# dmitrykoval/vinum

Measured on AMD Instinct MI355X. Metric: rows/sec + achieved HBM GB/s, filter->group-by over 10^9-row Arrow batches, higher is better.
Workload: dtype f64/int64; 1 GPU; configs[2]: SELECT k,sum(v),avg(v) WHERE v>63.9921875 GROUP BY k; N=1e+09 rows/GPU, G=1e+08 int64 keys, s=0.5; rows_per_gpu=1000000000, groups=100000000, group_count_hint=none: the operator samples the keys (what the reference boundary allows), parallelism=batch-sharded x1

## Files before the change

vinum_amd/csrc/vnm_agg.hip:

```cpp
#include <memory>
#include <algorithm>
#include <cmath>
#include <cstdlib>
#include <vector>

#include "vnm_agg.hpp"

namespace vnm {

constexpr uint64_t EMPTY = ~0ULL;
constexpr uint64_t LOCKED = ~0ULL - 1;
constexpr int AGG_BLOCK = 1024;
#ifndef VNM_AGG_R
#define VNM_AGG_R 8
#endif
constexpr int AGG_ROWS_PER_THREAD = VNM_AGG_R;
constexpr int AGG_TILE = AGG_BLOCK * AGG_ROWS_PER_THREAD;
constexpr int AGG_LDS_BUDGET = 128 * 1024;
constexpr int AGG_MAX_PROBES = 48;
constexpr int OG_BLOCK = 256;

struct GTable {
    uint64_t* tag;
    uint64_t* keyw;
// ... 197 lines not shown
            continue;
        }
        if (t == EMPTY) {
            uint64_t expected = EMPTY;
            if (__hip_atomic_compare_exchange_strong(&g.tag[h], &expected, LOCKED, __ATOMIC_RELAXED, __ATOMIC_RELAXED,
                                                     __HIP_MEMORY_SCOPE_AGENT)) {
                for (int i = 0; i < g.kwt; i++) st_agent(&g.keyw[(uint64_t)i * g.stride + h], kw[i]);
                asm volatile("s_waitcnt vmcnt(0)" ::: "memory");
                st_agent(&g.tag[h], tagv);
                atomicAdd(newc, 1u);
                return h;
            }
            continue;
        }
        if (t == LOCKED) continue;
        h = (h + 1) & mask;
    }
}

__device__ __forceinline__ void fold_new(const GTable& g, unsigned* s_new) {
    unsigned v = atomicExch(s_new, 0u);
    if (v) atomicAdd(&g.ctl[2], (unsigned long long)v);
}

__device__ __forceinline__ bool op_value(const AccOp& op, const vnm_dcol* cols, int64_t row, uint64_t* out) {
    if (op.kind == A_COUNT_ROWS) { *out = 1; return true; }
    const vnm_dcol& c = cols[op.col];
    if (!col_valid(c, row)) return false;
    switch (op.kind) {
        case A_COUNT_VALID: *out = 1; return true;
        case A_SUM_F64: *out = (uint64_t)__double_as_longlong(col_f64(c, row)); return true;
        case A_SUM_I64: *out = (uint64_t)col_i64(c, row); return true;
        case A_SUM_LO32: *out = (uint64_t)col_i64(c, row) & 0xFFFFFFFFULL; return true;
        case A_SUM_HI32S: *out = (uint64_t)(col_i64(c, row) >> 32); return true;
        case A_SUM_HI32U: *out = (uint64_t)col_i64(c, row) >> 32; return true;
        default:
            if (type_is_float(c.type)) *out = enc_f64(col_f64(c, row));
            else if (type_is_unsigned(c.type)) *out = (uint64_t)col_i64(c, row);
            else *out = enc_i64(col_i64(c, row));
            return true;
    }
}

__device__ __forceinline__ bool table_has_room(const AggArgs& a, unsigned* s_new) {
    fold_new(a.g, s_new);
    unsigned long long fill = __hip_atomic_load(&a.g.ctl[2], __ATOMIC_RELAXED, __HIP_MEMORY_SCOPE_AGENT);
    if ((int64_t)fill + a.margin > a.fill_limit) {
        __hip_atomic_store(&a.g.ctl[1], 1ULL, __ATOMIC_RELAXED, __HIP_MEMORY_SCOPE_AGENT);
        return false;
    }
    return true;
}

#include "vnm_agg_scan.inc"

#include "vnm_agg_tuple.inc"

#include "vnm_agg_onegroup.inc"

#include "vnm_agg_table.inc"

#include "vnm_agg_part.inc"

#include "vnm_agg_pack.inc"

#include "vnm_agg_dense.inc"

#include "vnm_agg_finalize.inc"

}

using namespace vnm;

struct DensePending {
    DFinalArgs df;
    int tb = 0, levels = 0, p1 = 0, fsplits = 1;
    int64_t nfinal = 0;
    int64_t dstride = 0;
    int64_t rows = 0;
    bool x_known = true;
    uint32_t x_inv = 0, x_exp = 0;
    bool exact_ok() const { return x_known && exact_adds_proved(((unsigned long long)x_exp << 32) | x_inv, rows); }
    std::vector<DSet> sets;
    std::vector<void*> blocks;
    DSet* dsets = nullptr;
    DTabSlot* table = nullptr;
    ~DensePending() { for (void* b : blocks) pool_free(b); pool_free(table); pool_free(dsets); }
};
constexpr size_t DP_MAX_SETS = 512;
struct DScanPending {
    DFinalArgs df{};
    DScanTable t{};
    int slots = 0;
    uint64_t* part_sum = nullptr;
    float* part_lo = nullptr;
    uint32_t* part_cnt = nullptr;
    unsigned long long* flags = nullptr;
    ~DScanPending() { pool_free(t.sum); pool_free(t.lo); pool_free(t.cnt); pool_free(part_sum); pool_free(part_lo); pool_free(part_cnt); pool_free(flags); }
};

struct vnm_agg {
    AggPlan plan;
    FuncOut outs[AGG_MAX_FUNCS];
    int n_funcs = 0;
    int func_col[AGG_MAX_FUNCS];
    int col_first_func[AGG_MAX_COLS];
    bool single = false;
    Predicate pred{};
    bool pred_set = false;
    int pred_op = 0, pred_is_float = 0;
    double pred_dval = 0;
    int64_t pred_ival = 0;
    int64_t hint = 0;
    GTable g{};
    bool have_table = false;
    int64_t rows_seen = 0;
    uint64_t* dkey = nullptr;
    uint64_t* dacc = nullptr;
    int64_t dstride = 0;
    int64_t n_groups = -1;
    std::vector<uint64_t> h_key, h_acc;
    bool host_ready = false;
    uint64_t* run_key = nullptr;
    uint64_t* run_acc = nullptr;
    int64_t run_stride = 0, run_n = 0;
    bool have_run = false;
    bool result_is_run = false;
    bool estimated = false;
    int64_t merge_stride = 0;
    unsigned long long* run_dir = nullptr;
    int64_t run_nfin = 0;
    vnm_agg* inner = nullptr;
    bool pack_tried = false;
    bool key_only_failed = false;
    int dense_state = 0;
    DenseMap dmap{};
    int64_t dense_span = 0;
    uint64_t dense_rlo = 0, dense_rhi = 0;
    bool rank_aligned = false;
    struct DensePending* pending = nullptr;
    double heavy_share = 0.0;
    int key_out_type = -1;
    std::vector<std::pair<int64_t, void*>> widened;
    bool widen_in[AGG_MAX_FUNCS] = {};
    bool any_widen_in = false;
    bool pred_lit_rounded = false;
    int pred_user_is_float = 0;
    double pred_user_dval = 0.0;
    int64_t pred_user_ival = 0;
    int fx_state = 0, fx_qe = 0;
    bool pack_null_seen = false;
    bool pring_off = false;
    bool fx_narrow = false;
    int fxn_state = 0, fxn_qe[3] = {0, 0, 0};
    bool null_inputs_seen = false;
    bool count8_off = false;
    int count_cb = 0;
    struct DScanPending* scan_pending = nullptr;
    bool dense_by_bound = false;
    bool range_given = false;
    int expr_col = -1;
    std::vector<vnm_expr_ins> expr_prog;
    int expr_ncols = 0;
    bool expr_fusable = false;
    bool expr_active = false;
    ExprProg expr_dev{};
    PackParams pack{};
    int c_funcs[AGG_MAX_FUNCS], c_in_types[AGG_MAX_FUNCS], c_in_flags[AGG_MAX_FUNCS], c_in_col_ids[AGG_MAX_FUNCS];
    bool c_has_ids = false;
    TDict tdict{};
    int64_t widest_est = 0;
    unsigned long long* tnext = nullptr;
    bool tuple_mode = false;
    std::vector<vnm_agg*> parts;
    std::vector<std::vector<int>> part_funcs;
    bool split_tried = false;
    bool async = false;
    struct QBatch { int64_t nrows; vnm_dcol key, col, pred; std::vector<vnm_dcol> ins; int64_t seq; };
    bool q_multi = false;
    std::vector<QBatch> q;
    int64_t q_rows = 0;
    bool q_pred_is_v = false;
    const std::vector<QBatch>* segs_active = nullptr;
    const uint8_t* kn_valid = nullptr;
    int64_t kn_off = 0;
    bool kn_failed = false;
    std::vector<VSeg> seg_host;
    struct vnm_agg_exact* ex = nullptr;
    bool child = false;
    int64_t seq = 0;
    int64_t cur_seq = -1;
};

namespace {

int table_alloc(vnm_agg* h, GTable* g, uint64_t cap, hipStream_t s) {
    memset(g, 0, sizeof(*g));
    g->cap = cap;
    g->stride = cap + 2;
    g->kwt = h->single || h->plan.n_keys == 0 ? 0 : h->plan.n_keys + 1;
    g->n_words = h->plan.n_words;
    g->tag = (uint64_t*)pool_alloc(g->stride * 8);
    g->acc = (uint64_t*)pool_alloc(g->stride * 8 * (size_t)g->n_words);
    g->ctl = (unsigned long long*)pool_alloc(64);
    if (g->kwt) g->keyw = (uint64_t*)pool_alloc(g->stride * 8 * (size_t)g->kwt);
    if (!g->tag || !g->acc || !g->ctl || (g->kwt && !g->keyw)) return 1;
    VNM_HIP(hipMemsetAsync(g->tag, 0xFF, g->stride * 8, s));
    VNM_HIP(hipMemsetAsync(g->ctl, 0, 64, s));
    for (int w = 0; w < g->n_words; w++) {
        const uint64_t init = merge_init(h->plan.merge[w]);
        if (init == 0 || init == ~0ULL) VNM_HIP(hipMemsetAsync(g->acc + (size_t)w * g->stride, init ? 0xFF : 0, g->stride * 8, s));
        else {
            fill_u64_kernel<<<(int)std::min<uint64_t>((g->stride + 255) / 256, (uint64_t)device_info().num_cus * 8), 256, 0, s>>>(g->acc + (size_t)w * g->stride, init, (int64_t)g->stride);
            VNM_HIP(hipGetLastError());
        }
    }
    return 0;
}

void table_free(GTable* g) {
    pool_free(g->tag);
    pool_free(g->acc);
    pool_free(g->keyw);
    pool_free(g->ctl);
    memset(g, 0, sizeof(*g));
}

uint64_t pow2_at_least(uint64_t x) {
    uint64_t p = 1;
    while (p < x) p <<= 1;
    return p;
}

int lds_slots_for(const AggPlan& p, int budget = AGG_LDS_BUDGET) {
    int per_slot = 8 * (1 + p.n_words);
    int s = 1;
    while ((s * 2 + 2) * per_slot <= budget) s *= 2;
    if (s > 8192) s = 8192;
    return s;
}

int table_grow(vnm_agg* h, uint64_t new_cap, hipStream_t s) {
    GTable old = h->g, ng;
    VNM_TRY(table_alloc(h, &ng, new_cap, s));
    MergeArgs m{};
    m.plan = h->plan;
    m.g = ng;
    m.n = (int64_t)old.stride;
    m.src_is_table = 1;
    m.src_stride = 1;
    m.src_tag = old.tag;
    m.src_cap = (int64_t)old.cap;
    for (int j = 0; j < old.kwt; j++) m.src_key[j] = old.keyw + (size_t)j * old.stride;
    for (int w = 0; w < old.n_words; w++) m.src_acc[w] = old.acc + (size_t)w * old.stride;
    int grid = device_info().num_cus * 8;
    agg_merge_kernel<<<grid, 256, 0, s>>>(m);
    VNM_HIP(hipGetLastError());
    VNM_HIP(hipStreamSynchronize(s));
    table_free(&old);
    h->g = ng;
    return 0;
}

int ensure_table(vnm_agg* h, int64_t nrows, hipStream_t s, bool rows_only = false) {
    if (h->have_table) return 0;
    uint64_t cap;
    if (h->plan.n_keys == 0) cap = 2;
    else {
        uint64_t want = h->hint > 0 ? (uint64_t)h->hint * 2 : (uint64_t)1 << 22;
        if ((h->hint <= 0 || rows_only) && (uint64_t)nrows * 2 < want) want = (uint64_t)(nrows > 512 ? nrows : 512) * 2;
        if (rows_only && want > (1ULL << 20)) want = 1ULL << 20;
        cap = pow2_at_least(want < 1024 ? 1024 : want);
    }
    VNM_TRY(table_alloc(h, &h->g, cap, s));
    h->have_table = true;
    return 0;
}

void invalidate_result(vnm_agg* h) {
    if (!h->result_is_run) {
        pool_free(h->dkey);
        pool_free(h->dacc);
    }
    h->result_is_run = false;
    h->dkey = h->dacc = nullptr;
    h->n_groups = -1;
    h->host_ready = false;
}

int64_t env_i64(const char* name, int64_t dflt) {
    const char* v = getenv(name);
    return v ? (int64_t)atoll(v) : dflt;
}

void drop_run(vnm_agg* h) {
    pool_free(h->run_key);
    pool_free(h->run_acc);
    pool_free(h->run_dir);
    h->run_dir = nullptr;
    h->run_nfin = 0;
    h->run_key = h->run_acc = nullptr;
    h->have_run = false;
    h->run_n = h->run_stride = 0;
}

int estimate_groups(vnm_agg* h, const vnm_dcol& key, int64_t nrows, int64_t* est, hipStream_t s, int64_t* tier0_lb = nullptr) {
// ... 866 lines not shown
```

vinum_amd/csrc/vnm_agg_dense.inc:

```

constexpr int DP_TBITS_MIN = 11, DP_TBITS_MAX = 13;
constexpr int DP_MAX_BITS = DP_TBITS_MAX + 18;

struct DenseMap {
    uint64_t lo_u;
    uint64_t sign;
    uint32_t mul;
    uint32_t mul_inv;
    uint32_t mask;
    int bits;
};

__device__ __forceinline__ uint64_t dense_key_of(const DenseMap& m, uint32_t codep) {
    const uint32_t code = (codep * m.mul_inv) & m.mask;
    return (m.lo_u + code) ^ m.sign;
}

struct DPartArgs {
    DenseMap map;
    const uint64_t* kp;
    const double* vp;
    const double* pp;
    int has_pred, pred_is_v, op;
    double thr;
    int64_t nrows;
    const VSeg* segs;
    int nseg;
    int64_t nsub;
    const double* vp2;
    const double* in_vals2;
    double* out_vals2;
    const uint8_t* kvalid;
    int64_t koff;
    uint64_t* nk_tag;
    uint64_t* nk_rows;
    uint64_t* nk_valid;
    uint64_t* nk_sum;
    int64_t nk_lo_stride;
    int has_expr;
    ExprProg expr;
    const double* in_vals;
    const uint32_t* in_codes;
    const uint32_t* in_counts;
    int64_t in_cap;
    int in_regions, in_split;
    int64_t in_pstride, in_rstride;
    int nt_store;
    int ready_list;
    int producer_major;
    int in_bits;
    double* out_vals;
    void* out_codes;
    uint32_t* out_counts;
    int64_t out_cap;
    int nparts;
    int out_bits;
    int in_pairs;
    unsigned long long* flags;
    ulonglong2* spill;
    int64_t spill_cap;
    const uint8_t* vvalid;
    int64_t voff;
    uint64_t* nspill;
    int64_t nspill_cap;
    double fx_q, fx_inv_q;
    int64_t fx_lim;
};
constexpr uint32_t DP_NULL32 = 0x80000000u;
__device__ __forceinline__ bool fx_encode(double v, double inv_q, int64_t* m, int64_t lim = 2147483647LL) {
    const double MAGIC = 6755399441055744.0;
    const double t = v * inv_q;
    const double u = t + MAGIC;
    const int64_t mm = (int64_t)(__double_as_longlong(u) - __double_as_longlong(MAGIC));
    *m = mm;
    return (u - MAGIC == t) && mm >= -lim && mm <= lim && __double_as_longlong(v) != (long long)0x8000000000000000ULL;
}
__device__ __forceinline__ double fx_bits(int64_t m) { return __longlong_as_double((long long)m); }
__device__ __forceinline__ int64_t fx_of(double carried) { return (int64_t)__double_as_longlong(carried); }
__device__ __forceinline__ void fx_expand(int64_t total, double q, double* hi, double* lo) {
    const double h = (double)total;
    const double l = (double)(total - (int64_t)h);
    *hi = h * q; *lo = l * q;
}

__device__ __forceinline__ void dense_spill(const DPartArgs& a, uint64_t key, double v, bool isnull = false) {
    if (isnull) {
        const unsigned long long pos = atomicAdd(&a.flags[3], 1ULL);
        if ((int64_t)pos < a.nspill_cap) a.nspill[pos] = key;
        else __hip_atomic_store(&a.flags[0], 1ULL, __ATOMIC_RELAXED, __HIP_MEMORY_SCOPE_AGENT);
        return;
    }
    const unsigned long long pos = atomicAdd(&a.flags[2], 1ULL);
    if ((int64_t)pos < a.spill_cap) a.spill[pos] = make_ulonglong2(key, (unsigned long long)__double_as_longlong(v));
    else __hip_atomic_store(&a.flags[0], 1ULL, __ATOMIC_RELAXED, __HIP_MEMORY_SCOPE_AGENT);
}
__device__ __forceinline__ void dense_spill_wave(const DPartArgs& a, bool want, uint64_t key, double v) {
    const unsigned long long m = __ballot(want);
    if (!m) return;
    const int lane = threadIdx.x & 63;
    const int leader = __ffsll((long long)m) - 1;
    unsigned long long base = 0;
    if (lane == leader) base = atomicAdd(&a.flags[2], (unsigned long long)__popcll(m));
    base = __shfl(base, leader);
    if (want) {
        const unsigned long long pos = base + (unsigned long long)__popcll(m & ((1ULL << lane) - 1ULL));
        if ((int64_t)pos < a.spill_cap) a.spill[pos] = make_ulonglong2(key, (unsigned long long)__double_as_longlong(v));
        else __hip_atomic_store(&a.flags[0], 1ULL, __ATOMIC_RELAXED, __HIP_MEMORY_SCOPE_AGENT);
    }
}
template <typename CT>
__device__ __forceinline__ CT dense_rem(uint32_t c, uint32_t remmask) {
    return (CT)((c & remmask) | ((c >> 31) << (sizeof(CT) * 8 - 1)));
}
template <typename CT>
__device__ __forceinline__ uint32_t dense_rem_code(CT r) { return (uint32_t)r & ((1u << (sizeof(CT) * 8 - 1)) - 1u); }
template <typename CT>
__device__ __forceinline__ bool dense_rem_null(CT r) { return ((uint32_t)r >> (sizeof(CT) * 8 - 1)) != 0; }

template <bool FROM_ROWS, typename CT, bool HAS_VAL = true, bool VN = false>
__global__ __launch_bounds__(PT_BLOCK) void dpart_scatter_kernel(DPartArgs a) {
    __shared__ double stage_v[HAS_VAL ? PT_TILE : 1];
    __shared__ uint32_t stage_c[PT_TILE];
    __shared__ uint32_t cnt[PT_MAXP], off[PT_MAXP], cursor[PT_MAXP];
    __shared__ uint32_t s_total;
    __shared__ uint32_t wtot[PT_MAXP / 64];
    const int tid = threadIdx.x;
    const int lane = tid & 63;
    const int np = a.nparts;
    const int npad = np < 64 ? 64 : np;
    const uint32_t remmask = (1u << a.out_bits) - 1u;
    for (int i = tid; i < PT_MAXP; i += PT_BLOCK) { cnt[i] = 0; cursor[i] = 0; }
    __syncthreads();

    int64_t out_base, out_stride;
    int64_t ntiles = 0;
    uint32_t prefix = 0;
    if (FROM_ROWS) {
        if (a.producer_major) { out_base = (int64_t)blockIdx.x * np; out_stride = 1; }
        else { out_base = blockIdx.x; out_stride = gridDim.x; }
        ntiles = (a.nrows + PT_TILE - 1) / PT_TILE;
    } else {
        const int pin = blockIdx.x / a.in_split, g = blockIdx.x % a.in_split;
        out_base = (int64_t)pin * np * a.in_split + g; out_stride = a.in_split;
        prefix = (uint32_t)pin << a.in_bits;
    }
    double* const ov = a.out_vals;
    CT* const oc = (CT*)a.out_codes;

    auto process_tile = [&](auto&& get_item, auto&& prefetch_next) {
        uint32_t myc[PT_ITEMS], myr[PT_ITEMS];
        double myv[PT_ITEMS];
#pragma unroll
        for (int k = 0; k < PT_ITEMS; k++) {
            myr[k] = 0xFFFFFFFFu;
            uint32_t c; double v;
            if (get_item(k, &c, &v)) {
                myc[k] = c;
                if (HAS_VAL) myv[k] = v;
                myr[k] = atomicAdd(&cnt[(c & ~DP_NULL32) >> a.out_bits], 1u);
            }
        }
        prefetch_next();
        __syncthreads();
        if (tid < npad) {
            uint32_t c = cnt[tid], inc = c;
#pragma unroll
            for (int d = 1; d < 64; d <<= 1) { uint32_t o = __shfl_up(inc, d); if (lane >= d) inc += o; }
            off[tid] = inc - c;
            if (lane == 63) wtot[tid >> 6] = inc;
        }
        __syncthreads();
        if (tid < npad) {
            uint32_t add = 0;
            for (int w = 0; w < (tid >> 6); w++) add += wtot[w];
            off[tid] += add;
            if (tid == npad - 1) s_total = off[tid] + cnt[tid];
        }
        __syncthreads();
#pragma unroll
        for (int k = 0; k < PT_ITEMS; k++) {
            if (myr[k] != 0xFFFFFFFFu) {
                const uint32_t pos = off[(myc[k] & ~DP_NULL32) >> a.out_bits] + myr[k];
                if (HAS_VAL) stage_v[pos] = myv[k];
                stage_c[pos] = myc[k];
            }
        }
        __syncthreads();
        const uint32_t total = s_total;
#pragma unroll
        for (int q = 0; q < PT_ITEMS; q++) {
            const uint32_t i = (uint32_t)q * PT_BLOCK + tid;
            bool lost = false;
            uint32_t c = 0;
            if (i < total) {
                c = stage_c[i];
                const uint32_t p = (c & ~DP_NULL32) >> a.out_bits;
                const uint32_t j = cursor[p] + (i - off[p]);
                if (j < (uint32_t)a.out_cap) {
                    const int64_t at = (out_base + (int64_t)p * out_stride) * a.out_cap + j;
                    if (a.nt_store) {
                        if (HAS_VAL) __builtin_nontemporal_store(stage_v[i], &ov[at]);
                        __builtin_nontemporal_store(dense_rem<CT>(c, remmask), &oc[at]);
                    } else {
                        if (HAS_VAL) ov[at] = stage_v[i];
                        oc[at] = dense_rem<CT>(c, remmask);
                    }
                } else lost = true;
            }
            if (lost && (c >> 31)) { dense_spill(a, dense_key_of(a.map, prefix | (c & ~DP_NULL32)), 0.0, true); lost = false; }
            dense_spill_wave(a, lost, dense_key_of(a.map, prefix | (c & ~DP_NULL32)), HAS_VAL && lost ? stage_v[i] : 0.0);
        }
        __syncthreads();
        if (tid < np) { cursor[tid] += cnt[tid]; cnt[tid] = 0; }
        __syncthreads();
    };

    if (FROM_ROWS) {
        ulonglong2 kk[PT_PAIRS];
        double2 vv[PT_PAIRS], pv[PT_PAIRS];
        uint8_t vb[VN ? PT_PAIRS : 1];
        auto load_rows = [&](int64_t tile) {
            const int64_t base = tile * PT_TILE;
            if (tile < ntiles && base + PT_TILE <= a.nrows) {
#pragma unroll
                for (int u = 0; u < PT_PAIRS; u++) {
                    const int64_t r = base + (int64_t)u * 2 * PT_BLOCK + 2 * tid;
                    kk[u] = *(const ulonglong2*)(a.kp + r);
                    if (HAS_VAL) vv[u] = a.has_expr ? expr_eval2(a.expr, r) : *(const double2*)(a.vp + r);
                    if (a.has_pred && !a.pred_is_v) pv[u] = *(const double2*)(a.pp + r);
                    if (VN) vb[VN ? u : 0] = (uint8_t)(a.vvalid[(a.voff + r) >> 3] >> ((a.voff + r) & 7));
                }
            }
        };
        load_rows(blockIdx.x);
        for (int64_t tile = blockIdx.x; tile < ntiles; tile += gridDim.x) {
            const int64_t base = tile * PT_TILE;
            const bool full = base + PT_TILE <= a.nrows;
            process_tile([&](int k, uint32_t* c, double* v) -> bool {
                const int u = k >> 1, el = k & 1;
                const int64_t r = base + (int64_t)u * 2 * PT_BLOCK + 2 * tid + el;
                if (r >= a.nrows) return false;
                uint64_t key; double val, p;
                bool isnull = false;
                if (full) {
                    key = el ? kk[u].y : kk[u].x;
                    val = HAS_VAL ? (el ? vv[u].y : vv[u].x) : 0.0;
                    p = a.pred_is_v ? val : (a.has_pred ? (el ? pv[u].y : pv[u].x) : 0.0);
                    if (VN) isnull = !((vb[VN ? u : 0] >> el) & 1);
                } else {
                    key = a.kp[r]; val = HAS_VAL ? (a.has_expr ? expr_eval1(a.expr, r) : a.vp[r]) : 0.0; p = a.has_pred ? (a.pred_is_v ? val : a.pp[r]) : 0.0;
                    if (VN) isnull = !((a.vvalid[(a.voff + r) >> 3] >> ((a.voff + r) & 7)) & 1);
                }
                if (VN && isnull && a.pred_is_v) return false;
                if (a.has_pred && !cmp_apply<double>(a.op, p, a.thr)) return false;
                const uint64_t d = (key ^ a.map.sign) - a.map.lo_u;
                if (d > (uint64_t)a.map.mask) { dense_spill(a, key, val, isnull); return false; }
                *c = (((uint32_t)d * a.map.mul) & a.map.mask) | (isnull ? DP_NULL32 : 0u);
                *v = isnull ? 0.0 : val;
                return true;
            }, [&]() { load_rows(tile + gridDim.x); });
        }
    } else {
        __shared__ uint32_t rstart[PT_MAX_REGIONS + 1];
        const int pin = blockIdx.x / a.in_split;
        const int per_max = (a.in_regions + a.in_split - 1) / a.in_split;
        const int g = blockIdx.x % a.in_split;
        const int first = g * per_max;
        const int per = first + per_max <= a.in_regions ? per_max : (a.in_regions > first ? a.in_regions - first : 0);
        const int64_t region0 = (int64_t)pin * a.in_pstride + (int64_t)first * a.in_rstride;
        if (tid == 0) {
            uint32_t run = 0;
            for (int rj = 0; rj < per; rj++) { rstart[rj] = run; run += (a.in_counts[region0 + rj * a.in_rstride] + 1) / 2; }
            rstart[per] = run;
        }
        __syncthreads();
        const uint32_t total_in = rstart[per];
        double2 ev[PT_PAIRS];
        uint2 ec[PT_PAIRS];
        uint32_t ok[PT_PAIRS];
        int reg[PT_PAIRS];
#pragma unroll
        for (int k = 0; k < PT_PAIRS; k++) reg[k] = 0;
        auto load_entries = [&](uint32_t t0) {
#pragma unroll
            for (int k = 0; k < PT_PAIRS; k++) {
                const uint32_t v = t0 + (uint32_t)k * PT_BLOCK + tid;
                ok[k] = 0;
                if (v < total_in) {
                    int lo = reg[k];
                    while (rstart[lo + 1] <= v) lo++;
                    reg[k] = lo;
                    const uint32_t e0 = 2u * (v - rstart[lo]);
                    const int64_t rg = region0 + lo * a.in_rstride;
                    const int64_t at = rg * a.in_cap + e0;
                    if (HAS_VAL) ev[k] = *(const double2*)(a.in_vals + at);
                    ec[k] = *(const uint2*)(a.in_codes + at);
                    ok[k] = e0 + 1 < a.in_counts[rg] ? 3u : 1u;
                }
            }
        };
        load_entries(0);
        for (uint32_t t0 = 0; t0 < total_in; t0 += PT_TILE / 2) {
            process_tile([&](int k, uint32_t* c, double* v) -> bool {
                const int u = k >> 1, el = k & 1;
                if (!((ok[u] >> el) & 1u)) return false;
                *c = el ? ec[u].y : ec[u].x;
                *v = HAS_VAL ? (el ? ev[u].y : ev[u].x) : 0.0;
                return true;
            }, [&]() { load_entries(t0 + PT_TILE / 2); });
        }
    }
    if (tid < np) a.out_counts[out_base + (int64_t)tid * out_stride] = cursor[tid] < (uint32_t)a.out_cap ? cursor[tid] : (uint32_t)a.out_cap;
}

__device__ __forceinline__ void exact_track(double v, uint32_t& xinv, uint32_t& xexp) {
    const uint64_t b = (uint64_t)__double_as_longlong(v) & 0x7FFFFFFFFFFFFFFFULL;
    if (b == 0) return;
    const uint32_t hi = (uint32_t)(b >> 32), lo = (uint32_t)b;
    const uint32_t e = hi >> 20;
    const uint32_t mh = (hi & 0xFFFFFu) | (e ? 0x100000u : 0u);
    const uint32_t tz = lo ? (uint32_t)__builtin_ctz(lo) : 32u + (uint32_t)__builtin_ctz(mh);
    const uint32_t low = (e ? e : 1u) + tz;
    xinv = max(xinv, 0xFFFFu - low);
    xexp = max(xexp, e);
}
static inline bool exact_adds_proved(unsigned long long word, int64_t rows) {
    const uint32_t xinv = (uint32_t)word, xexp = (uint32_t)(word >> 32);
    if (xinv == 0 && xexp == 0) return true;
    if (xexp >= 2047) return false;
    int lg = 0;
    while (((int64_t)1 << lg) < rows) lg++;
    return (int64_t)lg + (int64_t)xexp <= (int64_t)(0xFFFFu - xinv);
}

constexpr int DR_FB = 16;
typedef double dr_v2 __attribute__((ext_vector_type(2)));
typedef uint32_t dr_u2 __attribute__((ext_vector_type(2)));
template <bool FROM_ROWS, typename CT, bool HAS_VAL, int DR_BLOCK, int DR_PAIRS, bool PV = false, bool VN = false, int MAXR = 0, bool SEG = false, bool KN = false,
          bool V2 = false, bool FX = false, bool W32 = false>
__global__ __launch_bounds__(DR_BLOCK) void dring_scatter_kernel(DPartArgs a, int ring_cap) {
    extern __shared__ uint64_t dr_lds[];
    static_assert(!FX || (HAS_VAL && !V2), "fixed-point entries: one value (VN: only where the filter drops the NULL rows, vn_fold)");
    static_assert(!W32 || FX, "32-bit entry words are fixed-point words");
    constexpr int FB = W32 ? 32 : DR_FB, EPL = FB / 8;
    constexpr int NE = 2 * DR_PAIRS;
    const int np = a.nparts;
    double* const rv = (double*)dr_lds;
    double* const rv2 = rv + (V2 ? (size_t)np * ring_cap : 0);
    CT* const rc = (CT*)(dr_lds + (HAS_VAL ? (size_t)np * ring_cap * (V2 ? 2 : 1) : 0));
    __shared__ uint32_t fill[PT_MAXP], head[PT_MAXP], cursor[PT_MAXP];
    __shared__ uint32_t s_retry[2];
    __shared__ uint32_t s_nready[2];
    __shared__ uint16_t ready[2][PT_MAXP];
    __shared__ uint32_t s_spill[3];
    const int tid = threadIdx.x;
    const uint32_t remmask = (1u << a.out_bits) - 1u;
    for (int i = tid; i < PT_MAXP; i += DR_BLOCK) { fill[i] = 0; head[i] = 0; cursor[i] = 0; }
    if (tid < 2) { s_retry[tid] = 0; s_nready[tid] = 0; }
    int ph = 0;
    const bool use_list = a.ready_list != 0;
    if (tid == 0) s_spill[0] = 0;
    __syncthreads();

    int64_t out_base, out_stride;
    uint32_t prefix = 0;
    if (FROM_ROWS) {
        if (a.producer_major) { out_base = (int64_t)blockIdx.x * np; out_stride = 1; }
        else { out_base = blockIdx.x; out_stride = gridDim.x; }
    } else {
        const int pin = blockIdx.x / a.in_split, g = blockIdx.x % a.in_split;
        out_base = (int64_t)pin * np * a.in_split + g; out_stride = a.in_split;
        prefix = (uint32_t)pin << a.in_bits;
    }
    double* const ov = a.out_vals;
    double* const ov2 = a.out_vals2;
    CT* const oc = (CT*)a.out_codes;
    const uint32_t ocap = (uint32_t)a.out_cap;

    auto insert = [&](uint32_t c, double v, double w2) -> bool {
        const uint32_t p = (c & ~DP_NULL32) >> a.out_bits;
        const uint32_t r = atomicAdd(&fill[p], 1u);
        if (r == (uint32_t)FB - 1u && use_list) ready[ph][atomicAdd(&s_nready[ph], 1u)] = (uint16_t)p;
        if (r >= (uint32_t)ring_cap) return false;
        uint32_t slot = head[p] + r;
        if (slot >= (uint32_t)ring_cap) slot -= ring_cap;
        if (W32) {
            ((uint32_t*)rv)[(size_t)p * ring_cap + slot] = ((uint32_t)(int32_t)fx_of(v) << a.out_bits) | (c & remmask);
            return true;
        }
        if (FX) {
            ((uint64_t*)rv)[(size_t)p * ring_cap + slot] = ((uint64_t)fx_of(v) << a.out_bits) | (uint64_t)(c & remmask);
            return true;
        }
        if (HAS_VAL) rv[(size_t)p * ring_cap + slot] = v;
        if (V2) rv2[(size_t)p * ring_cap + slot] = w2;
        rc[(size_t)p * ring_cap + slot] = dense_rem<CT>(c, remmask);
        return true;
    };
    auto fx_rem = [&](size_t li) -> uint32_t { return W32 ? ((const uint32_t*)rv)[li] & remmask : (uint32_t)(((const uint64_t*)rv)[li] & (uint64_t)remmask); };
    auto fx_val = [&](size_t li) -> double {
        return W32 ? (double)((int32_t)((const uint32_t*)rv)[li] >> a.out_bits) * a.fx_q : (double)((int64_t)((const uint64_t*)rv)[li] >> a.out_bits) * a.fx_q;
    };
    auto flush = [&](bool drain) {
        const int j = tid & 7;
        const bool listed = use_list && !drain;
        const int nwalk = listed ? (int)s_nready[ph] : np;
        for (int q = tid >> 3; q < nwalk; q += DR_BLOCK / 8) {
            const int p = listed ? (int)ready[ph][q] : q;
            uint32_t f = fill[p];
            if (f > (uint32_t)ring_cap) f = ring_cap;
            const uint32_t nb = drain ? (f + FB - 1) / FB : f / FB;
            if (nb == 0) continue;
            const uint32_t h = head[p], cur = cursor[p];
            const int64_t rbase = (out_base + (int64_t)p * out_stride) * a.out_cap;
            uint32_t done = 0, wrote = 0;
            for (uint32_t b = 0; b < nb; b++) {
                uint32_t src = h + b * FB;
                if (src >= (uint32_t)ring_cap) src -= ring_cap;
                const uint32_t n_here = f - b * FB < (uint32_t)FB ? f - b * FB : FB;
                const size_t li = (size_t)p * ring_cap + src + EPL * j;
                if (cur + wrote + FB <= ocap) {
                    const int64_t at = rbase + cur + wrote + EPL * j;
                    if ((uint32_t)(EPL * j) < n_here) {
                        if (W32) {
                            const dr_v2 x = *(const dr_v2*)((const uint32_t*)rv + li);
                            if (a.nt_store) __builtin_nontemporal_store(x, (dr_v2*)((uint32_t*)ov + at)); else *(dr_v2*)((uint32_t*)ov + at) = x;
                        } else if (HAS_VAL) {
                            const dr_v2 x = *(const dr_v2*)(rv + li);
                            if (a.nt_store) __builtin_nontemporal_store(x, (dr_v2*)(ov + at)); else *(dr_v2*)(ov + at) = x;
                        }
                        if (V2) {
                            const dr_v2 x2 = *(const dr_v2*)(rv2 + li);
                            if (a.nt_store) __builtin_nontemporal_store(x2, (dr_v2*)(ov2 + at)); else *(dr_v2*)(ov2 + at) = x2;
                        }
                        if (FX) {
                        } else if (sizeof(CT) == 4) {
                            const dr_u2 y = *(const dr_u2*)(rc + li);
                            if (a.nt_store) __builtin_nontemporal_store(y, (dr_u2*)(oc + at)); else *(dr_u2*)(oc + at) = y;
                        } else {
                            const uint32_t y = *(const uint32_t*)(rc + li);
                            if (a.nt_store) __builtin_nontemporal_store(y, (uint32_t*)(oc + at)); else *(uint32_t*)(oc + at) = y;
                        }
                    }
                    wrote += n_here;
                } else if (V2) {
                    if (j == 0) __hip_atomic_store(&a.flags[0], 1ULL, __ATOMIC_RELAXED, __HIP_MEMORY_SCOPE_AGENT);
                } else if (!drain && a.nspill == nullptr) {
                    const unsigned long long m = __ballot(j == 0);
                    const int lane = tid & 63;
                    const int leader = __ffsll((long long)m) - 1;
                    unsigned long long base = 0;
                    if (lane == leader) base = atomicAdd(&a.flags[2], (unsigned long long)__popcll(m) * FB);
                    base = __shfl(base, leader);
                    const unsigned long long pos = base + (unsigned long long)__popcll(m & ((1ULL << (lane - j)) - 1ULL)) * FB + EPL * j;
                    if ((int64_t)(pos + EPL) <= a.spill_cap) {
                        for (int e = 0; e < EPL; e++)
                            a.spill[pos + e] = make_ulonglong2(dense_key_of(a.map, prefix | (p << a.out_bits) | (FX ? fx_rem(li + e) : dense_rem_code<CT>(rc[FX ? 0 : li + e]))),
                                                               (unsigned long long)__double_as_longlong(FX ? fx_val(li + e) : (HAS_VAL ? rv[li + e] : 0.0)));
                    } else __hip_atomic_store(&a.flags[0], 1ULL, __ATOMIC_RELAXED, __HIP_MEMORY_SCOPE_AGENT);
                } else {
                    for (int e = 0; e < EPL; e++)
                        if ((uint32_t)(EPL * j + e) < n_here) {
                            if (FX) dense_spill(a, dense_key_of(a.map, prefix | (p << a.out_bits) | fx_rem(li + e)), fx_val(li + e));
                            else dense_spill(a, dense_key_of(a.map, prefix | (p << a.out_bits) | dense_rem_code<CT>(rc[FX ? 0 : li + e])), HAS_VAL ? rv[li + e] : 0.0,
                                             dense_rem_null<CT>(rc[FX ? 0 : li + e]));
                        }
                }
                done += n_here;
            }
            if (j == 0) {
                uint32_t nh = h + nb * FB;
                while (nh >= (uint32_t)ring_cap) nh -= ring_cap;
                head[p] = drain ? 0 : nh;
                fill[p] = f - done;
                cursor[p] = cur + wrote;
            }
        }
    };
    int maxr = MAXR;
    auto rounds = [&](const uint32_t (&c)[NE], const double (&v)[NE], const double (&w2)[V2 ? NE : 1], uint32_t okmask) {
        uint32_t pend = 0;
        int nr = 0;
#pragma unroll
        for (int e = 0; e < NE; e++) if (((okmask >> e) & 1u) && !insert(c[e], v[e], w2[V2 ? e : 0])) pend |= 1u << e;
        for (;;) {
            if (pend) s_retry[ph] = 1;
            __syncthreads();
            flush(false);
            if (tid == 0) { s_retry[ph ^ 1] = 0; s_nready[ph ^ 1] = 0; }
            __syncthreads();
            const bool again = s_retry[ph] != 0;
            ph ^= 1;
            if (!again) break;
            if (MAXR > 0 && ++nr >= maxr) {
                uint32_t mine = 0;
#pragma unroll
                for (int e = 0; e < NE; e++) {
                    if (((pend >> e) & 1u) && (c[e] >> 31)) {
                        dense_spill(a, dense_key_of(a.map, prefix | (c[e] & ~DP_NULL32)), 0.0, true);
                        pend &= ~(1u << e);
                    }
                }
                mine = (uint32_t)__popc(pend);
                uint32_t at = mine ? atomicAdd(&s_spill[0], mine) : 0u;
                __syncthreads();
                if (tid == 0) {
                    const unsigned long long base = atomicAdd(&a.flags[2], (unsigned long long)s_spill[0]);
                    s_spill[1] = (uint32_t)base; s_spill[2] = (uint32_t)(base >> 32);
                }
                __syncthreads();
                const unsigned long long base = ((unsigned long long)s_spill[2] << 32) | s_spill[1];
#pragma unroll
                for (int e = 0; e < NE; e++) {
                    if ((pend >> e) & 1u) {
                        const unsigned long long pos = base + at++;
                        if ((int64_t)pos < a.spill_cap)
                            a.spill[pos] = make_ulonglong2(dense_key_of(a.map, prefix | c[e]),
                                                           (unsigned long long)__double_as_longlong(FX ? (double)fx_of(v[e]) * a.fx_q : (HAS_VAL ? v[e] : 0.0)));
                        else __hip_atomic_store(&a.flags[0], 1ULL, __ATOMIC_RELAXED, __HIP_MEMORY_SCOPE_AGENT);
                    }
                }
                __syncthreads();
                if (tid == 0) s_spill[0] = 0;
                maxr = MAXR - 1;
                break;
            }
#pragma unroll
            for (int e = 0; e < NE; e++) if (((pend >> e) & 1u) && insert(c[e], v[e], w2[V2 ? e : 0])) pend &= ~(1u << e);
        }
    };

    double nk_hi = -0.0, nk_lo = 0.0;
    uint32_t nk_cnt = 0;
    constexpr bool XT = FROM_ROWS && HAS_VAL && !V2 && !FX;
    uint32_t xinv = 0, xexp = 0;
    bool fx_bad = false;
    if (FROM_ROWS && !SEG) {
        const int64_t sub = (int64_t)NE * DR_BLOCK;
        const int64_t nsub = (a.nrows + sub - 1) / sub;
        const int64_t nfull = a.nrows / sub;
        ulonglong2 kk[DR_PAIRS];
        double2 vv[DR_PAIRS], pv[PV ? DR_PAIRS : 1], vv2[V2 ? DR_PAIRS : 1];
        uint32_t vbits = 0;
        uint32_t kbits = 0;
        auto load_sub = [&](int64_t st) {
            if (st < nfull) {
                if (VN) vbits = 0;
                if (KN) kbits = 0;
#pragma unroll
                for (int u = 0; u < DR_PAIRS; u++) {
                    const int64_t r = st * sub + (int64_t)u * 2 * DR_BLOCK + 2 * tid;
                    kk[u] = *(const ulonglong2*)(a.kp + r);
                    if (HAS_VAL) vv[u] = *(const double2*)(a.vp + r);
                    if (V2) vv2[V2 ? u : 0] = *(const double2*)(a.vp2 + r);
                    if (PV) pv[u] = *(const double2*)(a.pp + r);
                    if (VN) vbits |= (((uint32_t)a.vvalid[(a.voff + r) >> 3] >> ((a.voff + r) & 7)) & 3u) << (2 * u);
                    if (KN) kbits |= (((uint32_t)a.kvalid[(a.koff + r) >> 3] >> ((a.koff + r) & 7)) & 3u) << (2 * u);
                }
            }
        };
        load_sub(blockIdx.x);
        for (int64_t st = blockIdx.x; st < nsub; st += gridDim.x) {
            uint32_t c[NE]; double v[NE]; double w2[V2 ? NE : 1]; uint32_t okmask = 0;
#pragma unroll
            for (int e = 0; e < NE; e++) {
                const int u = e >> 1, el = e & 1;
                const int64_t r = st * sub + (int64_t)u * 2 * DR_BLOCK + 2 * tid + el;
                c[e] = 0; v[e] = 0.0;
                if (r >= a.nrows) continue;
                uint64_t key; double val, p, val2 = 0.0;
                bool isnull = false, keynull = false;
                if (st < nfull) {
                    if (KN) keynull = !((kbits >> e) & 1u);
                    key = el ? kk[u].y : kk[u].x;
                    val = HAS_VAL ? (el ? vv[u].y : vv[u].x) : 0.0;
                    if (V2) val2 = el ? vv2[V2 ? u : 0].y : vv2[V2 ? u : 0].x;
                    p = PV ? (el ? pv[PV ? u : 0].y : pv[PV ? u : 0].x) : val;
                    if (VN) isnull = !((vbits >> e) & 1u);
                } else {
                    key = a.kp[r]; val = HAS_VAL ? a.vp[r] : 0.0; p = a.has_pred ? (a.pred_is_v ? val : a.pp[r]) : 0.0;
                    if (V2) val2 = a.vp2[r];
                    if (VN) isnull = !((a.vvalid[(a.voff + r) >> 3] >> ((a.voff + r) & 7)) & 1);
                    if (KN) keynull = !((a.kvalid[(a.koff + r) >> 3] >> ((a.koff + r) & 7)) & 1);
                }
                if (VN && isnull && a.pred_is_v) continue;
                if (a.has_pred && !cmp_apply<double>(a.op, p, a.thr)) continue;
                if (KN && keynull) {
                    nk_cnt++;
                    const double t = nk_hi + val;
                    nk_lo += two_sum_err(nk_hi, val, t);
                    nk_hi = t;
                    continue;
                }
                const uint64_t d = (key ^ a.map.sign) - a.map.lo_u;
                if (d > (uint64_t)a.map.mask) {
                    if (V2) __hip_atomic_store(&a.flags[0], 1ULL, __ATOMIC_RELAXED, __HIP_MEMORY_SCOPE_AGENT);
                    else dense_spill(a, key, val, isnull);
                    continue;
                }
                c[e] = (((uint32_t)d * a.map.mul) & a.map.mask) | (VN && isnull ? DP_NULL32 : 0u);
                v[e] = VN && isnull ? 0.0 : val;
                if (FX) { int64_t m; if (!fx_encode(val, a.fx_inv_q, &m, a.fx_lim)) { fx_bad = true; continue; } v[e] = fx_bits(m); }
                if (V2) w2[V2 ? e : 0] = val2;
                if (XT) exact_track(v[e], xinv, xexp);
                okmask |= 1u << e;
            }
            load_sub(st + gridDim.x);
            rounds(c, v, w2, okmask);
        }
    } else if (FROM_ROWS) {
        const int64_t sub = (int64_t)NE * DR_BLOCK;
        struct Cur { const uint64_t* kp; const double* vp; const double* pp; const uint8_t* vvalid; int64_t voff; int64_t nrows; int64_t lst; };
        const int nseg = a.nseg;
        const VSegConst segs = seg_table(a.segs);
        const int64_t nsub = a.nsub;
        int sg = 0;
        auto locate = [&](int64_t st, Cur& c) {
            while (sg + 1 < nseg && st >= segs[sg + 1].first_tile) sg++;
            c.kp = segs[sg].kp; c.vp = (const double*)segs[sg].vp; c.pp = segs[sg].pp;
            c.vvalid = VN ? segs[sg].vvalid : nullptr; c.voff = VN ? segs[sg].voff : 0;
            c.nrows = segs[sg].nrows;
            c.lst = st - segs[sg].first_tile;
        };
        ulonglong2 kk[DR_PAIRS];
        double2 vv[DR_PAIRS], pv[PV ? DR_PAIRS : 1];
        uint32_t vbits = 0;
        auto load_sub = [&](const Cur& c) {
            if (c.lst < c.nrows / sub) {
                if (VN) vbits = 0;
#pragma unroll
                for (int u = 0; u < DR_PAIRS; u++) {
                    const int64_t r = c.lst * sub + (int64_t)u * 2 * DR_BLOCK + 2 * tid;
                    kk[u] = *(const ulonglong2*)(c.kp + r);
                    if (HAS_VAL) vv[u] = *(const double2*)(c.vp + r);
                    if (PV) pv[u] = *(const double2*)(c.pp + r);
                    if (VN) vbits |= (((uint32_t)c.vvalid[(c.voff + r) >> 3] >> ((c.voff + r) & 7)) & 3u) << (2 * u);
                }
            }
        };
        Cur cur{}, nxt{};
        if ((int64_t)blockIdx.x < nsub) { locate(blockIdx.x, cur); load_sub(cur); }
        for (int64_t st = blockIdx.x; st < nsub; st += gridDim.x) {
            uint32_t c[NE]; double v[NE]; uint32_t okmask = 0;
            const bool full = cur.lst < cur.nrows / sub;
#pragma unroll
            for (int e = 0; e < NE; e++) {
                const int u = e >> 1, el = e & 1;
                const int64_t r = cur.lst * sub + (int64_t)u * 2 * DR_BLOCK + 2 * tid + el;
                c[e] = 0; v[e] = 0.0;
                if (r >= cur.nrows) continue;
                uint64_t key; double val, p;
                bool isnull = false;
                if (full) {
                    key = el ? kk[u].y : kk[u].x;
                    val = HAS_VAL ? (el ? vv[u].y : vv[u].x) : 0.0;
                    p = PV ? (el ? pv[PV ? u : 0].y : pv[PV ? u : 0].x) : val;
                    if (VN) isnull = !((vbits >> e) & 1u);
                } else {
                    key = cur.kp[r]; val = HAS_VAL ? cur.vp[r] : 0.0; p = a.has_pred ? (a.pred_is_v ? val : cur.pp[r]) : 0.0;
                    if (VN) isnull = !((cur.vvalid[(cur.voff + r) >> 3] >> ((cur.voff + r) & 7)) & 1);
                }
                if (VN && isnull && a.pred_is_v) continue;
                if (a.has_pred && !cmp_apply<double>(a.op, p, a.thr)) continue;
                const uint64_t d = (key ^ a.map.sign) - a.map.lo_u;
                if (d > (uint64_t)a.map.mask) { dense_spill(a, key, val, isnull); continue; }
                c[e] = (((uint32_t)d * a.map.mul) & a.map.mask) | (VN && isnull ? DP_NULL32 : 0u);
                v[e] = VN && isnull ? 0.0 : val;
                if (FX) { int64_t m; if (!fx_encode(val, a.fx_inv_q, &m, a.fx_lim)) { fx_bad = true; continue; } v[e] = fx_bits(m); }
                if (XT) exact_track(v[e], xinv, xexp);
                okmask |= 1u << e;
            }
            if (st + gridDim.x < nsub) { locate(st + gridDim.x, nxt); load_sub(nxt); }
            const double w2[V2 ? NE : 1] = {};
            rounds(c, v, w2, okmask);
            cur = nxt;
        }
    } else {
        __shared__ uint32_t rstart[PT_MAX_REGIONS + 1];
        const int pin = blockIdx.x / a.in_split;
        const int per_max = (a.in_regions + a.in_split - 1) / a.in_split;
        const int g = blockIdx.x % a.in_split;
        const int first = g * per_max;
        const int per = first + per_max <= a.in_regions ? per_max : (a.in_regions > first ? a.in_regions - first : 0);
        const int64_t region0 = (int64_t)pin * a.in_pstride + (int64_t)first * a.in_rstride;
        if (tid == 0) {
            uint32_t run = 0;
            for (int rj = 0; rj < per; rj++) { rstart[rj] = run; run += (a.in_counts[region0 + rj * a.in_rstride] + 1) / 2; }
            rstart[per] = run;
        }
        __syncthreads();
        const uint32_t total_in = rstart[per];
        double2 ev[DR_PAIRS], ev2[V2 ? DR_PAIRS : 1];
        uint2 ec[DR_PAIRS];
        uint32_t okm = 0;
        int reg = 0;
        auto load_pairs = [&](uint32_t t0) {
            okm = 0;
#pragma unroll
            for (int u = 0; u < DR_PAIRS; u++) {
                const uint32_t v = t0 + (uint32_t)u * DR_BLOCK + tid;
                if (v < total_in) {
                    int lo = reg;
                    while (rstart[lo + 1] <= v) lo++;
                    reg = lo;
                    const uint32_t e0 = 2u * (v - rstart[lo]);
                    const int64_t rg = region0 + lo * a.in_rstride;
                    const int64_t at = rg * a.in_cap + e0;
                    if (HAS_VAL) ev[u] = *(const double2*)(a.in_vals + at);
                    if (V2) ev2[V2 ? u : 0] = *(const double2*)(a.in_vals2 + at);
                    if (!FX) ec[u] = *(const uint2*)(a.in_codes + at);
                    okm |= (e0 + 1 < a.in_counts[rg] ? 3u : 1u) << (2 * u);
                }
            }
        };
        load_pairs(0);
        for (uint32_t t0 = 0; t0 < total_in; t0 += DR_PAIRS * DR_BLOCK) {
            uint32_t c[NE]; double v[NE]; double w2[V2 ? NE : 1];
#pragma unroll
            for (int u = 0; u < DR_PAIRS; u++) {
                if (FX) {
                    const uint64_t w0 = (uint64_t)__double_as_longlong(ev[u].x), w1 = (uint64_t)__double_as_longlong(ev[u].y);
                    const uint64_t inmask = ((uint64_t)1 << a.in_bits) - 1;
                    c[2 * u] = (uint32_t)(w0 & inmask); c[2 * u + 1] = (uint32_t)(w1 & inmask);
                    v[2 * u] = fx_bits((int64_t)w0 >> a.in_bits); v[2 * u + 1] = fx_bits((int64_t)w1 >> a.in_bits);
                    continue;
                }
                c[2 * u] = ec[u].x; c[2 * u + 1] = ec[u].y;
                v[2 * u] = HAS_VAL ? ev[u].x : 0.0; v[2 * u + 1] = HAS_VAL ? ev[u].y : 0.0;
                if (V2) { w2[V2 ? 2 * u : 0] = ev2[V2 ? u : 0].x; w2[V2 ? 2 * u + 1 : 0] = ev2[V2 ? u : 0].y; }
            }
            const uint32_t okmask = okm;
            load_pairs(t0 + DR_PAIRS * DR_BLOCK);
            rounds(c, v, w2, okmask);
        }
    }
    flush(true);
    __syncthreads();
    if (tid < np) a.out_counts[out_base + (int64_t)tid * out_stride] = cursor[tid];
    if (FX && FROM_ROWS) { if (__syncthreads_or(fx_bad ? 1 : 0) && tid == 0) __hip_atomic_store(&a.flags[7], 1ULL, __ATOMIC_RELAXED, __HIP_MEMORY_SCOPE_AGENT); }
    if (XT) {
        if (tid < 2) s_spill[tid] = 0;
        __syncthreads();
        if (xinv) atomicMax(&s_spill[0], xinv);
        if (xexp) atomicMax(&s_spill[1], xexp);
        __syncthreads();
        if (tid < 2 && s_spill[tid]) atomicMax((uint32_t*)&a.flags[6] + tid, s_spill[tid]);
    }
    if (KN) {
        __shared__ uint64_t s_nk[3];
        __syncthreads();
        if (tid < 3) s_nk[tid] = tid == 0 ? F64_NEG_ZERO : 0;
        __syncthreads();
        if (nk_cnt) {
            l_add_f64c(&s_nk[0], 1, nk_hi);
            __hip_atomic_fetch_add((double*)&s_nk[1], nk_lo, __ATOMIC_RELAXED, __HIP_MEMORY_SCOPE_WORKGROUP);
            __hip_atomic_fetch_add(&s_nk[2], (uint64_t)nk_cnt, __ATOMIC_RELAXED, __HIP_MEMORY_SCOPE_WORKGROUP);
        }
        __syncthreads();
        if (tid == 0 && s_nk[2]) {
            if (ld_agent(a.nk_tag) == EMPTY) st_agent(a.nk_tag, 0);
            if (a.nk_rows) __hip_atomic_fetch_add(a.nk_rows, s_nk[2], __ATOMIC_RELAXED, __HIP_MEMORY_SCOPE_AGENT);
            if (a.nk_valid) __hip_atomic_fetch_add(a.nk_valid, s_nk[2], __ATOMIC_RELAXED, __HIP_MEMORY_SCOPE_AGENT);
            if (a.nk_sum) {
                if (a.nk_lo_stride) {
                    g_add_f64c(a.nk_sum, a.nk_lo_stride, __longlong_as_double((long long)s_nk[0]));
                    __hip_atomic_fetch_add((double*)(a.nk_sum + a.nk_lo_stride), __longlong_as_double((long long)s_nk[1]), __ATOMIC_RELAXED, __HIP_MEMORY_SCOPE_AGENT);
                } else __hip_atomic_fetch_add((double*)a.nk_sum, __longlong_as_double((long long)s_nk[0]) + __longlong_as_double((long long)s_nk[1]), __ATOMIC_RELAXED, __HIP_MEMORY_SCOPE_AGENT);
            }
        }
    }
}

__global__ void dnull_fold_kernel(const unsigned long long* scr, uint64_t* tag, uint64_t* rows, uint64_t* valid, uint64_t* sum, int64_t lo_stride) {
    if (threadIdx.x != 0 || blockIdx.x != 0) return;
    if (!(scr[1] | scr[2])) return;
    if (ld_agent(tag) == EMPTY) st_agent(tag, 0);
    if (rows) __hip_atomic_fetch_add(rows, scr[1], __ATOMIC_RELAXED, __HIP_MEMORY_SCOPE_AGENT);
    if (valid) __hip_atomic_fetch_add(valid, scr[2], __ATOMIC_RELAXED, __HIP_MEMORY_SCOPE_AGENT);
    if (sum) {
        if (lo_stride) {
            g_add_f64c(sum, lo_stride, __longlong_as_double((long long)scr[3]));
            __hip_atomic_fetch_add((double*)(sum + lo_stride), __longlong_as_double((long long)scr[4]), __ATOMIC_RELAXED, __HIP_MEMORY_SCOPE_AGENT);
        } else __hip_atomic_fetch_add((double*)sum, __longlong_as_double((long long)scr[3]), __ATOMIC_RELAXED, __HIP_MEMORY_SCOPE_AGENT);
    }
}

struct DSet {
    const double* vals; const void* codes; const uint32_t* counts;
    int64_t cap, pstride, rstride;
    int regions, pad;
};
__device__ __forceinline__ const double* dfin_words(const double* base, int64_t entries, bool w32) {
    return w32 ? (const double*)((const uint32_t*)base + entries) : base + entries;
}
constexpr int DF_MAX_OUT = 8;
enum { DF_RUN = 0, DF_COLS = 1, DF_TABLE = 2 };
enum { DF_KEY = 0, DF_SUM = 1, DF_AVG = 2, DF_COUNT = 3 };
struct DTabSlot { double sum; float lo; uint32_t cnt; };
struct DFinalArgs {
    int64_t pstride, rstride;
    DenseMap map;
    const double* vals;
    const void* codes;
    const uint32_t* counts;
    int64_t cap;
    int regions;
    int64_t nfinal;
    int w_rows, w_valid, w_sum, w_lo;
    uint64_t* dkey;
    uint64_t* dacc;
    int64_t dstride;
    unsigned long long* flags;
    int splits;
    uint64_t* part_sum;
    float* part_lo;
    uint32_t* part_cnt;
    int n_out;
    int out_kind[DF_MAX_OUT];
    int key_width;
    void* out_ptr[DF_MAX_OUT];
    DTabSlot* table;
    const DSet* sets;
    int nsets;
    int sub_bits, sub;
    int has_side;
    GTable side;
    const uint32_t* side_bloom;
    uint32_t side_bloom_mask;
    uint8_t* side_found;
    int64_t* null_pos;
    const double* vals2;
    int w_valid2, w_sum2, w_lo2;
    double fx_q;
    int fx_w32;
    int pack_n;
    int key_field[DF_MAX_OUT];
    int pack_shift[AGG_MAX_KEYS], pack_bits[AGG_MAX_KEYS];
    uint64_t pack_lo[AGG_MAX_KEYS];
};
__device__ __forceinline__ uint64_t df_key_cell(const DFinalArgs& a, int c, uint64_t key) {
    if (!a.pack_n) return key;
    const int f = a.key_field[c];
    return ((key >> a.pack_shift[f]) & ((1ULL << a.pack_bits[f]) - 1ULL)) + a.pack_lo[f];
}
__device__ __forceinline__ void df_store_cell(const DFinalArgs& a, int c, int64_t pos, uint64_t cell) {
    if (a.out_kind[c] == DF_KEY && a.key_width && a.key_width != 8) {
        if (a.key_width == 4) ((uint32_t*)a.out_ptr[c])[pos] = (uint32_t)cell;
        else if (a.key_width == 2) ((uint16_t*)a.out_ptr[c])[pos] = (uint16_t)cell;
        else ((uint8_t*)a.out_ptr[c])[pos] = (uint8_t)cell;
        return;
    }
    ((uint64_t*)a.out_ptr[c])[pos] = cell;
}
constexpr int DSIDE_BLOOM_BITS = 1 << 16;
__device__ __forceinline__ uint32_t dside_bloom_bit(uint64_t k, uint32_t mask) { return hash_u64(k ^ 0xD6E8FEB86659FD93ULL) & mask; }
__device__ __forceinline__ uint32_t dside_bloom_pattern(uint64_t k, uint32_t b) {
    const uint32_t h2 = hash_u64(k * 0x9E3779B97F4A7C15ULL + 0x632BE59BD9B4E019ULL);
    return (1u << (b & 31)) | (1u << ((h2 >> 7) & 31));
}
__device__ __forceinline__ void dside_merge(const DFinalArgs& a, const uint32_t* lb, uint64_t key, double& hi, double& lo, uint64_t& cnt) {
    const GTable& g = a.side;
    uint64_t slot = ~0ULL;
    if (key == EMPTY) { if (g.tag[g.cap] != EMPTY) slot = g.cap; }
    else {
        const uint32_t bb = dside_bloom_bit(key, a.side_bloom_mask);
        const uint32_t word = (lb && a.side_bloom_mask == DSIDE_BLOOM_BITS - 1) ? lb[bb >> 5] : a.side_bloom[bb >> 5];
        const uint32_t pat = dside_bloom_pattern(key, bb);
        if ((word & pat) != pat) return;
        const uint64_t mask = g.cap - 1;
        uint64_t h = hash_u64(key) & mask;
        for (uint64_t probes = 0; probes <= mask; probes++) {
            const uint64_t t = g.tag[h];
            if (t == key) { slot = h; break; }
            if (t == EMPTY) break;
            h = (h + 1) & mask;
        }
    }
    if (slot == ~0ULL) return;
    const int wc = a.w_rows >= 0 ? a.w_rows : a.w_valid;
    if (wc >= 0) cnt += g.acc[(uint64_t)wc * g.stride + slot];
    if (a.w_sum >= 0) {
        const double sh = __longlong_as_double((long long)g.acc[(uint64_t)a.w_sum * g.stride + slot]);
        const double t = hi + sh;
        lo += two_sum_err(hi, sh, t);
        if (a.w_lo >= 0) lo += __longlong_as_double((long long)g.acc[(uint64_t)a.w_lo * g.stride + slot]);
        hi = t;
    }
    a.side_found[slot] = 1;
}
__global__ __launch_bounds__(256) void dside_bloom_kernel(GTable g, uint32_t* bloom, uint32_t bmask) {
    const int64_t stride = (int64_t)gridDim.x * 256;
    for (int64_t slot = (int64_t)blockIdx.x * 256 + threadIdx.x; slot < (int64_t)g.cap; slot += stride) {
// ... 1083 lines not shown
            for (uint32_t i0 = 0; i0 < n; i0 += 64 * 4 * 2) {
                uint4 q[2];
#pragma unroll
                for (int u = 0; u < 2; u++) {
                    const uint32_t i = i0 + ((uint32_t)u * 64 + lane) * 4;
                    if (i < n) q[u] = *(const uint4*)(sc + i);
                }
#pragma unroll
                for (int u = 0; u < 2; u++) {
                    const uint32_t i = i0 + ((uint32_t)u * 64 + lane) * 4;
                    const uint32_t c4[4] = {q[u].x, q[u].y, q[u].z, q[u].w};
#pragma unroll
                    for (int k = 0; k < 4; k++) {
                        if (i + k >= n) continue;
                        const uint32_t code = c4[k];
                        if ((code >> tb8) != sub) continue;
                        const uint32_t b = code & ((1u << tb8) - 1u), sh = (b & (uint32_t)(PER - 1)) * (uint32_t)CB;
                        const uint32_t old = atomicAdd(&dc_tab[b >> PSH], 1u << sh);
                        over |= ((old >> sh) & CMASK) == CMASK;
                    }
                }
            }
        }
        if (over) s_over = 1;
        __syncthreads();
        if (s_over) {
            if (tid == 0) { __hip_atomic_store(&a.flags[5], 1ULL, __ATOMIC_RELAXED, __HIP_MEMORY_SCOPE_AGENT); __hip_atomic_store(&a.flags[0], 1ULL, __ATOMIC_RELAXED, __HIP_MEMORY_SCOPE_AGENT); }
            return;
        }
        uint32_t mine = 0;
        for (int i = tid; i < (1 << (tb8 - PSH)); i += 1024) {
            const uint32_t x = dc_tab[i];
            if (CB == 8) mine += ((x & 0xffu) != 0) + ((x & 0xff00u) != 0) + ((x & 0xff0000u) != 0) + ((x >> 24) != 0);
            else mine += ((x & 0xffffu) != 0) + ((x >> 16) != 0);
        }
        pa_block_add(&s_n, mine);
        __syncthreads();
        const uint32_t ngroups = s_n;
        __syncthreads();
        if (tid == 0) { s_base = atomicAdd(&a.flags[1], (unsigned long long)ngroups); s_n = 0; }
        __syncthreads();
        if ((int64_t)(s_base + ngroups) > a.dstride) {
            if (tid == 0) __hip_atomic_store(&a.flags[0], 1ULL, __ATOMIC_RELAXED, __HIP_MEMORY_SCOPE_AGENT);
            return;
        }
        const uint32_t prefix = ((uint32_t)p << (tb8 + sub_bits)) | (sub << tb8);
        for (int i0 = 0; i0 < (1 << tb8); i0 += 1024) {
            const int i = i0 + tid;
            const uint32_t cnt = (dc_tab[i >> PSH] >> ((i & (PER - 1)) * CB)) & CMASK;
            const bool occ = cnt != 0;
            const uint64_t b = __ballot(occ);
            uint32_t wbase = 0;
            if (lane == 0 && b) wbase = atomicAdd(&s_n, (uint32_t)__popcll(b));
            wbase = __shfl(wbase, 0);
            if (occ) {
                const uint64_t lt = lane == 0 ? 0ULL : (~0ULL >> (64 - lane));
                dgen_write_group(a, (int64_t)s_base + wbase + __popcll(b & lt), prefix | (uint32_t)i, cnt, nullptr);
            }
        }
        __syncthreads();
    }
}

struct DScanTable {
    double* sum;
    double* lo;
    unsigned long long* cnt;
};
__global__ __launch_bounds__(512) void dscan_accumulate_kernel(const uint64_t* part_sum, const float* part_lo, const uint32_t* part_cnt,
                                                                int splits, int slots, DScanTable t) {
    __shared__ double s_hi[8][64], s_lo[8][64];
    __shared__ unsigned long long s_cnt[8][64];
    const int li = threadIdx.x & 63, g = threadIdx.x >> 6;
    const int i = blockIdx.x * 64 + li;
    double hi = -0.0, lo = 0.0;
    unsigned long long cnt = 0;
    constexpr int U = 4;
    for (int sp0 = g; sp0 < splits; sp0 += 8 * U) {
        uint32_t c[U]; uint64_t xs[U]; float xl[U];
#pragma unroll
        for (int u = 0; u < U; u++) {
            const int sp = sp0 + 8 * u;
            c[u] = 0; xs[u] = 0; xl[u] = 0.0f;
            if (sp < splits && i < slots) {
                const size_t at = (size_t)sp * slots + i;
                c[u] = part_cnt[at]; xs[u] = part_sum[at]; xl[u] = part_lo[at];
            }
        }
#pragma unroll
        for (int u = 0; u < U; u++) {
            if (c[u] == 0) continue;
            cnt += c[u];
            const double x = __longlong_as_double((long long)xs[u]);
            const double s = hi + x;
            lo += two_sum_err(hi, x, s) + (double)xl[u];
            hi = s;
        }
    }
    s_hi[g][li] = hi; s_lo[g][li] = lo; s_cnt[g][li] = cnt;
    __syncthreads();
    if (g != 0 || i >= slots) return;
    for (int gg = 1; gg < 8; gg++) {
        const unsigned long long c = s_cnt[gg][li];
        if (c == 0) continue;
        cnt += c;
        const double x = s_hi[gg][li];
        const double s = hi + x;
        lo += two_sum_err(hi, x, s) + s_lo[gg][li];
        hi = s;
    }
    if (cnt == 0) return;
    const double old = t.sum[i], s = old + hi;
    t.lo[i] += two_sum_err(old, hi, s) + lo;
    t.sum[i] = s;
    t.cnt[i] += cnt;
}
__global__ __launch_bounds__(512) void dscan_emit_kernel(DFinalArgs a, int slots, DScanTable t) {
    __shared__ uint32_t s_n;
    __shared__ unsigned long long s_base;
    const int tid = threadIdx.x, lane = tid & 63;
    const int i = blockIdx.x * 512 + tid;
    if (tid == 0) s_n = 0;
    __syncthreads();
    const unsigned long long cnt = i < slots ? t.cnt[i] : 0ULL;
    const bool occ = cnt != 0;
    pa_block_add(&s_n, occ ? 1u : 0u);
    __syncthreads();
    const uint32_t ngroups = s_n;
    __syncthreads();
    if (tid == 0) { s_base = atomicAdd(&a.flags[1], (unsigned long long)ngroups); s_n = 0; }
    __syncthreads();
    if ((int64_t)(s_base + ngroups) > a.dstride) {
        if (tid == 0) __hip_atomic_store(&a.flags[0], 1ULL, __ATOMIC_RELAXED, __HIP_MEMORY_SCOPE_AGENT);
        return;
    }
    const uint64_t b = __ballot(occ);
    uint32_t wbase = 0;
    if (lane == 0 && b) wbase = atomicAdd(&s_n, (uint32_t)__popcll(b));
    wbase = __shfl(wbase, 0);
    if (occ) {
        const uint64_t lt = lane == 0 ? 0ULL : (~0ULL >> (64 - lane));
        const int64_t pos = (int64_t)s_base + wbase + __popcll(b & lt);
        const double hi = t.sum[i], lo = t.lo[i];
        a.dkey[pos] = dense_key_of(a.map, (uint32_t)i);
        a.dkey[a.dstride + pos] = 0;
        if (a.w_rows >= 0) a.dacc[(int64_t)a.w_rows * a.dstride + pos] = cnt;
        if (a.w_valid >= 0) a.dacc[(int64_t)a.w_valid * a.dstride + pos] = cnt;
        if (a.w_sum >= 0) a.dacc[(int64_t)a.w_sum * a.dstride + pos] = (uint64_t)__double_as_longlong(hi);
        if (a.w_lo >= 0) a.dacc[(int64_t)a.w_lo * a.dstride + pos] = (uint64_t)__double_as_longlong(lo);
        else if (a.w_sum >= 0) a.dacc[(int64_t)a.w_sum * a.dstride + pos] = (uint64_t)__double_as_longlong(fsum2(hi, lo));
    }
}

__global__ __launch_bounds__(256) void fx_sample_kernel(const double* vals, int64_t nrows, int64_t m, unsigned long long* out) {
    __shared__ uint32_t sx[2];
    if (threadIdx.x < 2) sx[threadIdx.x] = 0;
    __syncthreads();
    const int64_t stride = (int64_t)gridDim.x * blockDim.x;
    uint32_t xinv = 0, xexp = 0;
    for (int64_t i = (int64_t)blockIdx.x * blockDim.x + threadIdx.x; i < m; i += stride) exact_track(vals[(int64_t)(((__int128)i * nrows) / m)], xinv, xexp);
    if (xinv) atomicMax(&sx[0], xinv);
    if (xexp) atomicMax(&sx[1], xexp);
    __syncthreads();
    if (threadIdx.x < 2 && sx[threadIdx.x]) atomicMax((uint32_t*)out + threadIdx.x, sx[threadIdx.x]);
}

__global__ __launch_bounds__(256) void dense_sample_range_kernel(const uint64_t* keys, int64_t nrows, int64_t m, uint64_t sign,
                                                                 unsigned long long* out, const uint8_t* kvalid, int64_t koff) {
    __shared__ unsigned long long smn[4], smx[4];
    const int64_t stride = (int64_t)gridDim.x * blockDim.x;
    uint64_t mn = ~0ULL, mx = 0;
    for (int64_t i = (int64_t)blockIdx.x * blockDim.x + threadIdx.x; i < m; i += stride) {
        const int64_t row = (int64_t)(((__int128)i * nrows) / m);
        if (!key_row_valid(kvalid, koff, row)) continue;
        const uint64_t ku = keys[row] ^ sign;
        mn = ku < mn ? ku : mn;
        mx = ku > mx ? ku : mx;
    }
#pragma unroll
    for (int o = 32; o > 0; o >>= 1) {
        const uint64_t omn = __shfl_xor(mn, o), omx = __shfl_xor(mx, o);
        mn = omn < mn ? omn : mn;
        mx = omx > mx ? omx : mx;
    }
    if ((threadIdx.x & 63) == 0) { smn[threadIdx.x >> 6] = mn; smx[threadIdx.x >> 6] = mx; }
    __syncthreads();
    if (threadIdx.x == 0) {
        for (int w = 1; w < 4; w++) { mn = smn[w] < mn ? smn[w] : mn; mx = smx[w] > mx ? smx[w] : mx; }
        atomicMin(&out[0], (unsigned long long)mn);
        atomicMax(&out[1], (unsigned long long)mx);
    }
}
```

vinum_amd/csrc/vnm_agg_fxn.inc:

```
constexpr int FXN_MAXV = 3;
constexpr int FXN_BLOCK = 1024;
constexpr int FXN_FB = 16;
typedef uint32_t fxn_u4 __attribute__((ext_vector_type(4)));

struct VSegN { const uint64_t* kp; const double* vp[FXN_MAXV]; const double* pp; int64_t nrows; int64_t first_tile; };
typedef const VSegN __attribute__((address_space(4)))* VSegNConst;

struct FxnArgs {
    DenseMap map;
    const uint64_t* kp;
    const double* vp[FXN_MAXV];
    const double* pp;
    int has_pred, pred_col, op;
    double thr;
    int64_t nrows;
    const VSegN* segs;
    int nseg;
    int64_t nsub;
    double inv_q[FXN_MAXV];
    const fxn_u4* in_ent;
    const uint32_t* in_counts;
    int64_t in_cap;
    int in_regions, in_split;
    int in_bits;
// ... 242 lines not shown
    const int tid = threadIdx.x, lane = tid & 63;
    const int R = a.regions;
    const int64_t nwork = a.nfinal;
    int buf = 0;
    if ((int64_t)blockIdx.x < nwork) for (int r = tid; r < R && r < MAXR; r += BLOCK) s_cnt[0][r] = a.counts[(int64_t)blockIdx.x * R + r];
    __syncthreads();
    auto first_region = [&](const uint32_t* cnt) { int r = 0; while (r < R && cnt[r] == 0) r++; return r; };
    fxn_u4 pa = fxn_u4{0u, 0u, 0u, 0u}, pb = pa;
    uint32_t na = 0, ia = 0, nb = 0, ib = 0;
    auto load_chunk = [&](int64_t f, int rj, uint32_t ci, uint32_t n, fxn_u4* p) {
        const uint32_t i = ci + tid;
        if (i < n) *p = a.ent[(f * R + rj) * a.cap + i];
    };
    int rj = 0; uint32_t ci = 0;
    bool have = false;
    if ((int64_t)blockIdx.x < nwork) {
        rj = first_region(s_cnt[0]);
        have = rj < R;
        if (have) { na = s_cnt[0][rj]; ia = 0; load_chunk(blockIdx.x, rj, 0, na, &pa); ci = BLOCK; }
    }
    for (int64_t w = blockIdx.x; w < nwork; w += gridDim.x) {
        const int64_t f = w, wn = w + gridDim.x;
        for (int i = tid; i < SLOTS; i += BLOCK) {
#pragma unroll
            for (int v = 0; v < NV; v++) lsum[v][i] = 0ULL;
            lcnt[i] = 0;
        }
        if (tid == 0) s_n = 0;
        uint32_t cnext[CQ];
        if (wn < nwork) {
#pragma unroll
            for (int q = 0; q < CQ; q++) { const int r = q * BLOCK + tid; cnext[q] = r < R ? a.counts[wn * R + r] : 0u; }
        }
        __syncthreads();
        const uint32_t* cnt = s_cnt[buf];
        while (have) {
            int rn = rj; uint32_t cin = ci;
            while (rn < R && cin >= cnt[rn]) { rn++; cin = 0; }
            const bool more = rn < R;
            if (more) { nb = cnt[rn]; ib = cin; load_chunk(f, rn, cin, nb, &pb); }
            if (ia + tid < na) {
                const uint32_t slot = pa.w & (SLOTS - 1);
                atomicAdd(&lsum[0][slot], (unsigned long long)(long long)(int32_t)pa.x);
                if (NV > 1) atomicAdd(&lsum[NV > 1 ? 1 : 0][slot], (unsigned long long)(long long)(int32_t)pa.y);
                if (NV > 2) atomicAdd(&lsum[NV > 2 ? 2 : 0][slot], (unsigned long long)(long long)(int32_t)pa.z);
                atomicAdd(&lcnt[slot], 1u);
            }
            have = more;
            if (more) { pa = pb; na = nb; ia = ib; rj = rn; ci = cin + BLOCK; }
        }
        if (wn < nwork) {
#pragma unroll
            for (int q = 0; q < CQ; q++) { const int r = q * BLOCK + tid; if (r < R) s_cnt[buf ^ 1][r] = cnext[q]; }
        }
        __syncthreads();
        if (wn < nwork) {
            const uint32_t* cn2 = s_cnt[buf ^ 1];
            rj = first_region(cn2);
            have = rj < R;
            if (have) { na = cn2[rj]; ia = 0; load_chunk(wn, rj, 0, na, &pa); ci = BLOCK; }
        }
        buf ^= 1;
        uint32_t mine = 0;
#pragma unroll
        for (int q = 0; q < SLOTS / BLOCK; q++) mine += lcnt[q * BLOCK + tid] != 0 ? 1u : 0u;
        pa_block_add(&s_n, mine);
        __syncthreads();
        const uint32_t ngroups = s_n;
        __syncthreads();
        if (tid == 0) { s_base = atomicAdd(&a.flags[1], (unsigned long long)ngroups); s_n = 0; }
        __syncthreads();
        if ((int64_t)(s_base + ngroups) > a.dstride) {
            if (tid == 0) __hip_atomic_store(&a.flags[0], 1ULL, __ATOMIC_RELAXED, __HIP_MEMORY_SCOPE_AGENT);
            return;
        }
        for (int i0 = 0; i0 < SLOTS; i0 += BLOCK) {
            const int i = i0 + tid;
            const uint32_t gc = lcnt[i];
            const bool occ = gc != 0;
            const uint64_t b = __ballot(occ);
            uint32_t wbase = 0;
            if (lane == 0 && b) wbase = atomicAdd(&s_n, (uint32_t)__popcll(b));
            wbase = __shfl(wbase, 0);
            if (occ) {
                const uint64_t lt = lane == 0 ? 0ULL : (~0ULL >> (64 - lane));
                const int64_t pos = (int64_t)s_base + wbase + __popcll(b & lt);
                a.dkey[pos] = dense_key_of(a.map, ((uint32_t)f << TB) | (uint32_t)i);
                a.dkey[a.dstride + pos] = 0;
                for (int k = 0; k < a.n_cnt; k++) a.dacc[(int64_t)a.w_cnt[k] * a.dstride + pos] = gc;
#pragma unroll
                for (int v = 0; v < NV; v++) {
                    if (a.w_sum[v] < 0) continue;
                    double hi, lo;
                    fx_expand((long long)lsum[v][i], a.q[v], &hi, &lo);
                    a.dacc[(int64_t)a.w_sum[v] * a.dstride + pos] = (uint64_t)__double_as_longlong(hi);
                    a.dacc[(int64_t)(a.w_sum[v] + 1) * a.dstride + pos] = (uint64_t)__double_as_longlong(lo);
                }
            }
        }
        __syncthreads();
    }
}

int dense_fxn_aggregate(vnm_agg* h, int64_t nrows, const vnm_dcol* keys, const vnm_dcol* inputs, const vnm_dcol* pred, hipStream_t s) {
    if (env_i64("VNM_DENSE_FXN", 1) == 0 || h->fxn_state < 0) return 2;
    const AggPlan& pl = h->plan;
    const int NV = pl.n_cols;
    if (!h->single || pl.n_keys != 1 || NV < 2 || NV > FXN_MAXV || h->rank_aligned || h->kn_valid || h->expr_col >= 0 || h->dense_state != 1) return 2;
    auto plain8 = [](const vnm_dcol& c) { return !c.validity && (c.offset & 1) == 0 && ((uintptr_t)c.values & 15) == 0; };
    if ((keys[0].type != VNM_I64 && keys[0].type != VNM_U64) || !plain8(keys[0])) return 2;
    FxnFinalArgs fa{};
    for (int v = 0; v < FXN_MAXV; v++) fa.w_sum[v] = -1;
    for (int o = 0; o < pl.n_ops; o++) {
        const AccOp& op = pl.ops[o];
        if (op.kind == A_COUNT_ROWS || op.kind == A_COUNT_VALID) { if (fa.n_cnt > FXN_MAXV) return 2; fa.w_cnt[fa.n_cnt++] = op.word; }
        else if (op.kind == A_SUM_F64 && op.col >= 0 && op.col < NV && fa.w_sum[op.col] < 0 && pl.merge[op.word] == M_ADD_F64C) fa.w_sum[op.col] = op.word;
        else return 2;
    }
    if (fa.n_cnt == 0) return 2;
    vnm_dcol cols[FXN_MAXV];
    for (int c = 0; c < NV; c++) {
        cols[c] = inputs[h->col_first_func[c]];
        if (cols[c].type != VNM_F64 || !plain8(cols[c])) return 2;
    }
    int pred_col = -1;
    double thr = 0.0;
    if (h->pred_set) {
        if (!pred || pred->type != VNM_F64 || !plain8(*pred)) return 2;
        for (int c = 0; c < NV; c++) if (pred->values == cols[c].values && pred->offset == cols[c].offset) pred_col = c;
        thr = h->pred_is_float ? h->pred_dval : (double)h->pred_ival;
    }
    const std::vector<vnm_agg::QBatch>* q = h->segs_active;
    if (q) {
        for (const auto& b : *q) {
            if (b.ins.size() != (size_t)h->n_funcs || !plain8(b.key)) return 2;
            for (int c = 0; c < NV; c++) if (b.ins[h->col_first_func[c]].type != VNM_F64 || !plain8(b.ins[h->col_first_func[c]])) return 2;
            if (h->pred_set) {
                if (b.pred.type != VNM_F64 || !plain8(b.pred)) return 2;
                const vnm_dcol& pc = pred_col >= 0 ? b.ins[h->col_first_func[pred_col]] : b.pred;
                if (pred_col >= 0 && (b.pred.values != pc.values || b.pred.offset != pc.offset)) return 2;
            }
        }
    } else if (nrows < env_i64("VNM_FXN_MIN_ROWS", (int64_t)1 << 24)) return 2;
    const int cus = device_info().num_cus;
    if (h->fxn_state == 0) {
        h->fxn_state = -1;
        unsigned long long* d = (unsigned long long*)pool_alloc(64);
        if (!d) return 1;
        unsigned long long got[FXN_MAXV] = {0, 0, 0};
        VNM_HIP(hipMemsetAsync(d, 0, 8 * FXN_MAXV, s));
        const int64_t srows = q ? (*q)[0].nrows : nrows;
        const int64_t m = std::min<int64_t>(srows, 1 << 16);
        for (int c = 0; c < NV; c++)
            fx_sample_kernel<<<(int)std::min<int64_t>((m + 255) / 256, 256), 256, 0, s>>>((const double*)cols[c].values + cols[c].offset, srows, m, d + c);
        VNM_HIP(hipGetLastError());
        VNM_HIP(hipMemcpyAsync(got, d, 8 * FXN_MAXV, hipMemcpyDeviceToHost, s));
        VNM_HIP(hipStreamSynchronize(s));
        pool_free(d);
        bool ok = true;
        for (int c = 0; c < NV && ok; c++) {
            const uint32_t xinv = (uint32_t)got[c], xexp = (uint32_t)(got[c] >> 32);
            if (xinv == 0 && xexp == 0) { h->fxn_qe[c] = -16; continue; }
            ok = false;
            if (xexp >= 2047) break;
            const int L = (int)(0xFFFFu - xinv) - 1075, E = (int)xexp - 1022;
            const int spare = 31 - (E - L);
            if (spare < 0) break;
            int qe = L - spare / 2;
            if (qe > 0) qe = 0;
            if (qe < -1000 || E - qe > 31) break;
            h->fxn_qe[c] = qe;
            ok = true;
        }
        if (!ok) return 2;
        h->fxn_state = 1;
    }
    const DenseMap& mp = h->dmap;
    int tb = (int)env_i64("VNM_FXN_TBITS", 11);
    tb = std::max(10, std::min(12, tb));
    if (mp.bits - tb > 16) tb = mp.bits - 16;
    if (tb > 12 || mp.bits - tb < 5) return 2;
    const int pbits = mp.bits - tb;
    const int levels = pbits > 8 ? 2 : 1;
    const int p1 = levels == 2 ? pbits / 2 : pbits, p2 = pbits - p1;
    const int np1 = 1 << p1, np2 = levels == 2 ? 1 << p2 : 0;
    auto ring_cap_for = [&](int np) { int cap = (int)((size_t)128 * 1024 / ((size_t)np * 16) / FXN_FB) * FXN_FB; return std::min(cap, 128); };
    const int rcap1 = ring_cap_for(np1), rcap2 = levels == 2 ? ring_cap_for(np2) : 0;
    if (rcap1 < 2 * FXN_FB || (levels == 2 && rcap2 < 2 * FXN_FB)) return 2;
    const int pairs1 = 2;
    const int64_t sub1 = (int64_t)2 * pairs1 * FXN_BLOCK;
    PoolScope seg_pool;
    std::vector<VSegN> hseg;
    int64_t nsub = (nrows + sub1 - 1) / sub1;
    const VSegN* dseg = nullptr;
    if (q) {
        hseg.resize(q->size());
        int64_t t = 0;
        for (size_t i = 0; i < q->size(); i++) {
            const auto& b = (*q)[i];
            VSegN& g = hseg[i];
            g.kp = (const uint64_t*)b.key.values + b.key.offset;
            for (int c = 0; c < FXN_MAXV; c++) { const vnm_dcol& x = b.ins[h->col_first_func[c < NV ? c : 0]]; g.vp[c] = (const double*)x.values + x.offset; }
            g.pp = h->pred_set ? (const double*)b.pred.values + b.pred.offset : nullptr;
            g.nrows = b.nrows; g.first_tile = t;
            t += (b.nrows + sub1 - 1) / sub1;
        }
        nsub = t;
        VSegN* d = (VSegN*)seg_pool.take(hseg.size() * sizeof(VSegN));
        if (!d) return 1;
        VNM_HIP(hipMemcpyAsync(d, hseg.data(), hseg.size() * sizeof(VSegN), hipMemcpyHostToDevice, s));
        dseg = d;
    }
    const int grid1 = (int)std::min<int64_t>((int64_t)cus * 2, nsub);
    int split2 = std::max(2, (grid1 + PT_MAX_REGIONS - 1) / PT_MAX_REGIONS);
    split2 = std::max(split2, std::min(grid1, (cus * 2 + np1 - 1) / np1));
    const int64_t subs_per_wg = (nsub + grid1 - 1) / grid1;
    const int64_t rows_per_wg = subs_per_wg * sub1;
    int64_t cap1 = ((rows_per_wg / np1 + rows_per_wg / np1 / 5 + 512) + 15) & ~15LL;
    if (((cap1 / 16) & 1) == 0) cap1 += 16;
    if (levels == 1 && grid1 > 512) return 2;
    PoolScope pool;
    struct SyncOnExit { hipStream_t s; ~SyncOnExit() { (void)hipStreamSynchronize(s); } } sync_on_exit{s};
    unsigned long long* flags = (unsigned long long*)pool.take(128);
    fxn_u4* e1 = (fxn_u4*)pool.take((size_t)np1 * grid1 * cap1 * 16);
    uint32_t* n1 = (uint32_t*)pool.take((size_t)np1 * grid1 * 4);
    if (!flags || !e1 || !n1) return 1;
    if (h->pending && complete_pending(h, s)) return 1;
    if (h->have_run && merge_run_into_table(h, s)) return 1;
    VNM_HIP(hipMemsetAsync(flags, 0, 128, s));
    FxnArgs d1{};
    d1.map = mp;
    d1.kp = (const uint64_t*)keys[0].values + keys[0].offset;
    for (int c = 0; c < FXN_MAXV; c++) { const vnm_dcol& x = cols[c < NV ? c : 0]; d1.vp[c] = (const double*)x.values + x.offset; d1.inv_q[c] = std::ldexp(1.0, -h->fxn_qe[c < NV ? c : 0]); }
    d1.pp = h->pred_set ? (const double*)pred->values + pred->offset : nullptr;
    d1.has_pred = h->pred_set ? 1 : 0; d1.pred_col = pred_col; d1.op = h->pred_op; d1.thr = thr;
    d1.nrows = nrows; d1.segs = dseg; d1.nseg = q ? (int)q->size() : 0; d1.nsub = nsub;
    d1.out_ent = e1; d1.out_counts = n1; d1.out_cap = cap1; d1.out_pstride = grid1;
    d1.nparts = np1; d1.out_bits = mp.bits - p1;
    d1.flags = flags; d1.ready_list = (int)env_i64("VNM_FXN_READY_LIST", 1) & 1;
    const bool pv = h->pred_set && pred_col < 0;
    {
        KernelTimer timer("agg_part_scatter1", s);
        const size_t lds = (size_t)np1 * rcap1 * 16;
#define VNM_FXN1(NV_, SEG_, PV_)                                                                                        \
    do {                                                                                                              \
        VNM_HIP(hipFuncSetAttribute((const void*)fxn_scatter_kernel<true, NV_, 2, SEG_, PV_>, hipFuncAttributeMaxDynamicSharedMemorySize, (int)lds)); \
        fxn_scatter_kernel<true, NV_, 2, SEG_, PV_><<<grid1, FXN_BLOCK, lds, s>>>(d1, rcap1);                          \
    } while (0)
#define VNM_FXN1_S(NV_) do { if (q) { if (pv) VNM_FXN1(NV_, true, true); else VNM_FXN1(NV_, true, false); } else { if (pv) VNM_FXN1(NV_, false, true); else VNM_FXN1(NV_, false, false); } } while (0)
        if (NV == 2) VNM_FXN1_S(2); else VNM_FXN1_S(3);
#undef VNM_FXN1_S
#undef VNM_FXN1
        VNM_HIP(hipGetLastError());
    }
    const fxn_u4* fin_e = e1; const uint32_t* fin_n = n1;
    int64_t fin_cap = cap1;
    int fin_regions = grid1;
    if (levels == 2) {
        const int64_t per_pg = (int64_t)grid1 * rows_per_wg / np1 / split2;
        int64_t cap2 = ((per_pg / np2 + per_pg / np2 / 4 + 256) + 15) & ~15LL;
        if (((cap2 / 16) & 1) == 0) cap2 += 16;
        fxn_u4* e2 = (fxn_u4*)pool.take((size_t)np1 * np2 * split2 * cap2 * 16);
        uint32_t* n2 = (uint32_t*)pool.take((size_t)np1 * np2 * split2 * 4);
        if (!e2 || !n2) return 1;
        FxnArgs d2{};
        d2.map = mp;
        d2.in_ent = e1; d2.in_counts = n1; d2.in_cap = cap1; d2.in_regions = grid1; d2.in_split = split2; d2.in_bits = mp.bits - p1;
        d2.out_ent = e2; d2.out_counts = n2; d2.out_cap = cap2;
        d2.nparts = np2; d2.out_bits = tb;
        d2.flags = flags; d2.ready_list = ((int)env_i64("VNM_FXN_READY_LIST", 1) >> 1) & 1;
        {
            KernelTimer timer("agg_part_scatter2", s);
            const size_t lds = (size_t)np2 * rcap2 * 16;
            if (NV == 2) {
                VNM_HIP(hipFuncSetAttribute((const void*)fxn_scatter_kernel<false, 2, 2, false, false>, hipFuncAttributeMaxDynamicSharedMemorySize, (int)lds));
                fxn_scatter_kernel<false, 2, 2, false, false><<<np1 * split2, FXN_BLOCK, lds, s>>>(d2, rcap2);
            } else {
                VNM_HIP(hipFuncSetAttribute((const void*)fxn_scatter_kernel<false, 3, 2, false, false>, hipFuncAttributeMaxDynamicSharedMemorySize, (int)lds));
                fxn_scatter_kernel<false, 3, 2, false, false><<<np1 * split2, FXN_BLOCK, lds, s>>>(d2, rcap2);
            }
            VNM_HIP(hipGetLastError());
        }
        fin_e = e2; fin_n = n2; fin_cap = cap2; fin_regions = split2;
    }
    unsigned long long fl[8];
    VNM_HIP(hipMemcpyAsync(fl, flags, 64, hipMemcpyDeviceToHost, s));
    VNM_HIP(hipStreamSynchronize(s));
    if (fl[0] || fl[7]) {
        h->fxn_state = -1;
        route_note("dense:fixed_point_columns_failed", "%s: the batch takes the per-column route", fl[7] ? "a value that is not a 31-bit multiple of its column's quantum" : "a key outside the code range or an overflowing ring / region");
        return 2;
    }
    const int64_t dstride = std::min<int64_t>(h->dense_span, nrows) + 2;
    uint64_t* rk = (uint64_t*)pool.take((size_t)dstride * 8 * 2);
    uint64_t* ra = (uint64_t*)pool.take((size_t)dstride * 8 * pl.n_words);
    if (!rk || !ra) return 1;
    fa.map = mp;
    fa.ent = fin_e; fa.counts = fin_n; fa.cap = fin_cap; fa.regions = fin_regions; fa.nfinal = (int64_t)1 << pbits;
    for (int c = 0; c < FXN_MAXV; c++) fa.q[c] = std::ldexp(1.0, h->fxn_qe[c < NV ? c : 0]);
    fa.dkey = rk; fa.dacc = ra; fa.dstride = dstride; fa.flags = flags;
    {
        KernelTimer timer("agg_part_final", s);
#define VNM_FXNF(NV_, TB_)                                                                                             \
    do {                                                                                                              \
        const int blk = TB_ >= 12 ? 1024 : 512;                                                                       \
        int occ = 0;                                                                                                  \
        if (hipOccupancyMaxActiveBlocksPerMultiprocessor(&occ, (const void*)fxn_final_kernel<NV_, TB_>, blk, 0) != hipSuccess || occ < 1) occ = 1; \
// ... 20 lines not shown
```

vinum_amd/csrc/vnm_agg_routes.inc:

```
namespace {
template <class F>
int pick_bool(bool b, F&& f) { return b ? f(std::true_type{}) : f(std::false_type{}); }
template <int LO, int HI, class F>
int pick_int(int v, F&& f) {
    if constexpr (LO < HI) { if (v > LO) return pick_int<LO + 1, HI>(v, f); }
    return f(std::integral_constant<int, LO>{});
}
template <class F>
int pick_out(int out, F&& f) {
    if (out == DF_COLS) return f(std::integral_constant<int, DF_COLS>{});
    if (out == DF_TABLE) return f(std::integral_constant<int, DF_TABLE>{});
    return f(std::integral_constant<int, DF_RUN>{});
}
template <class K, class Q, class... A>
int launch_resident_as(K kernel, Q occ_kernel, int64_t work, int block, size_t lds, int occ_max, hipStream_t s, const A&... args) {
    if (lds) VNM_HIP(hipFuncSetAttribute((const void*)kernel, hipFuncAttributeMaxDynamicSharedMemorySize, (int)lds));
    int occ = 0;
    if (hipOccupancyMaxActiveBlocksPerMultiprocessor(&occ, (const void*)occ_kernel, block, lds) != hipSuccess || occ < 1) occ = 1;
    const int grid = (int)std::min<int64_t>(work, (int64_t)device_info().num_cus * std::min(occ, occ_max));
    kernel<<<grid, block, lds, s>>>(args...);
    return 0;
}
template <class K, class... A>
int launch_resident(K kernel, int64_t work, int block, size_t lds, int occ_max, hipStream_t s, const A&... args) {
    return launch_resident_as(kernel, kernel, work, block, lds, occ_max, s, args...);
}
template <class K, class... A>
int launch_dyn(K kernel, int grid, int block, size_t lds, hipStream_t s, const A&... args) {
    VNM_HIP(hipFuncSetAttribute((const void*)kernel, hipFuncAttributeMaxDynamicSharedMemorySize, (int)lds));
    kernel<<<grid, block, lds, s>>>(args...);
    return 0;
}
template <class K>
int launch_part_final(K kernel, int64_t work, size_t lds, hipStream_t s, const PartAggArgs& pa) {
    const int cus = device_info().num_cus;
    if (lds) VNM_HIP(hipFuncSetAttribute((const void*)kernel, hipFuncAttributeMaxDynamicSharedMemorySize, (int)lds));
    int grid = (int)std::min<int64_t>(work, (int64_t)cus * 4), occ = 0;
    if (hipOccupancyMaxActiveBlocksPerMultiprocessor(&occ, (const void*)kernel, PA_BLOCK, lds) == hipSuccess && occ > 0)
        grid = (int)std::min<int64_t>(work, (int64_t)cus * std::min(occ, (int)env_i64("VNM_PA_OCC", 8)));
    kernel<<<grid, PA_BLOCK, lds, s>>>(pa);
    return 0;
}

struct RingLaunch { int grid, cap, pairs; bool limit, seg, kn; hipStream_t s; };
constexpr int ring_flush_block(bool w32) { return w32 ? 32 : DR_FB; }
inline bool ring_one_round(int pairs, int nparts, int cap, bool w32) { return 2 * pairs * 1024 <= nparts * (cap - ring_flush_block(w32)); }
inline int ring_sub_tile_pairs(int want, bool pv, bool limit, int nparts, int cap, bool w32) {
    int pr = want >= 4 && !pv ? 4 : (want >= 2 ? 2 : 1);
    while (limit && pr > 1 && !ring_one_round(pr, nparts, cap, w32)) pr >>= 1;
    return pr;
}
inline int ring_cap_for(int np, size_t esize) {
    int cap = (int)((size_t)(env_i64("VNM_DENSE_RING_LDS", 128) * 1024) / ((size_t)np * esize) / DR_FB) * DR_FB;
    cap = std::min(cap, (int)env_i64("VNM_DENSE_RING_CAP", std::max(80, ((8192 / np + DR_FB + DR_FB - 1) / DR_FB) * DR_FB)));
    if (np < env_i64("VNM_DENSE_RING_MIN_NP", 32)) return 0;
    return cap >= 2 * DR_FB ? cap : 0;
}
inline int ring_cap_w32(int np) {
    const int cap = std::min(256, (int)((size_t)128 * 1024 / ((size_t)np * 4) / 32) * 32);
    return cap >= 64 ? cap : 0;
}

template <bool FR, typename CT, bool HV, int PR, bool PV, bool VN, int MAXR, bool SEG, bool KN, bool V2, bool FX, bool W32>
int launch_ring(int grid, const DPartArgs& d, int cap, hipStream_t s) {
    constexpr size_t esize = FX ? (W32 ? 4 : 8) : (HV ? (V2 ? 16 : 8) : 0) + sizeof(CT);
    const size_t lds = (((size_t)d.nparts * cap * esize) + 15) & ~(size_t)15;
    return launch_dyn(dring_scatter_kernel<FR, CT, HV, 1024, PR, PV, VN, MAXR, SEG, KN, V2, FX, W32>, grid, 1024, lds, s, d, cap);
}
template <bool FR, typename CT, bool HV, bool PV, bool VN, bool FX, bool W32, int PR>
int ring_scatter_pairs(const RingLaunch& r, const DPartArgs& d) {
    auto go = [&](auto lim, auto seg, auto kn) {
        return launch_ring<FR, CT, HV, PR, PV, VN, decltype(lim)::value ? 2 : 0, decltype(seg)::value, decltype(kn)::value, false, FX, W32>(r.grid, d, r.cap, r.s);
    };
    return pick_bool(r.limit && ring_one_round(PR, d.nparts, r.cap, W32), [&](auto lim) {
        if constexpr (FR && HV && !VN) {
            if (r.kn) return go(lim, std::false_type{}, std::true_type{});
            if (r.seg) return go(lim, std::true_type{}, std::false_type{});
        }
        return go(lim, std::false_type{}, std::false_type{});
    });
}
template <bool FR, typename CT, bool HV, bool PV, bool VN, bool FX = false, bool W32 = false>
int ring_scatter(const RingLaunch& r, const DPartArgs& d) {
    if constexpr (!PV) {
        if (r.pairs == 4) return ring_scatter_pairs<FR, CT, HV, PV, VN, FX, W32, 4>(r, d);
    }
    if (r.pairs >= 2) return ring_scatter_pairs<FR, CT, HV, PV, VN, FX, W32, 2>(r, d);
    return ring_scatter_pairs<FR, CT, HV, PV, VN, FX, W32, 1>(r, d);
}


int partitioned_aggregate(vnm_agg* h, const AggArgs& a, int64_t nrows, hipStream_t s, ulonglong2** spill_out = nullptr,
                          int64_t* n_spill_out = nullptr) {
    const int cus = device_info().num_cus;
    const int64_t l1_cap = env_i64("VNM_AGG_PART_L1_MAX", 256) * 512;
    const bool small_tables = a.part_generic && (size_t)(PA_SLOTS + 1) * 8 * (1 + h->plan.n_words) > 54 * 1024 &&
                              h->hint / 450 < l1_cap && getenv("VNM_AGG_NO_SMALL_TABLES") == nullptr;
    int pa_slots = small_tables ? PA_SLOTS / 2 : PA_SLOTS;
    while (a.part_generic && pa_slots > 256 && (size_t)(pa_slots + 1) * 8 * (1 + h->plan.n_words) > 150 * 1024) pa_slots /= 2;
    const int64_t per_final = env_i64("VNM_AGG_PART_GROUPS", 900 * pa_slots / PA_SLOTS);
    int64_t nfin = 2;
    while (nfin * per_final < h->hint) nfin *= 2;
    const int64_t l1_max = env_i64("VNM_AGG_PART_L1_MAX", 256);
    if (nfin > l1_max * 512) {
        if (h->hint / (l1_max * 512) > 1600 * pa_slots / PA_SLOTS) return 2;
        nfin = l1_max * 512;
    }
    const int E = a.part_wide ? 1 + h->plan.n_cols + (a.part_vmask ? 1 : 0) : 2;
    const bool wide = a.part_wide != 0;
    const int64_t tile1 = wide ? pw_tile(E) : PT_TILE;
    const size_t ebytes = (size_t)E * 8;
    const int levels = nfin > std::min<int64_t>(l1_max * 2, PT_MAXP) ? 2 : 1;
    const int np1 = levels == 2 ? (int)l1_max : (int)nfin;
    const int np2 = levels == 2 ? (int)(nfin / l1_max) : 0;
    const int grid1 = (int)std::min<int64_t>((int64_t)cus * 2, (nrows + tile1 - 1) / tile1);
    const int split2 = std::max(2, (grid1 + PT_MAX_REGIONS - 1) / PT_MAX_REGIONS);
    const int64_t tiles_per_wg = ((nrows + tile1 - 1) / tile1 + grid1 - 1) / grid1;
    const int64_t rows_per_wg = tiles_per_wg * tile1;
    const double slack = std::max(0.0, 4.5 / std::sqrt((double)std::max<int64_t>(per_final, 16) / 2.0));
    const int64_t cap1 = rows_per_wg / np1 + (int64_t)((double)(rows_per_wg / np1) * std::max(0.2, slack)) + 512;
    PoolScope pool;
    unsigned long long* flags = (unsigned long long*)pool.take(64);
    ulonglong2* e1 = (ulonglong2*)pool.take((size_t)np1 * grid1 * cap1 * ebytes);
    uint32_t* c1 = (uint32_t*)pool.take((size_t)np1 * grid1 * 4);
    if (!flags || !e1 || !c1) return 1;
    VNM_HIP(hipMemsetAsync(flags, 0, 64, s));
    const int64_t spill_cap = spill_out ? nrows / 2 + (1 << 20) : 0;
    ulonglong2* spill = spill_out ? (ulonglong2*)pool.take((size_t)spill_cap * (wide ? ebytes : 16)) : nullptr;
    if (spill_out && !spill) return 1;
    PartArgs p1{};
    p1.kp = (const uint64_t*)a.keys[0].values + a.keys[0].offset;
    p1.vp = h->plan.n_cols ? (const double*)a.cols[0].values + a.cols[0].offset : (const double*)p1.kp;
    p1.has_expr = a.has_expr; p1.expr = a.expr;
    p1.pp = h->pred_set ? (const double*)a.pred.values + a.pred.offset : nullptr;
    p1.has_pred = h->pred_set; p1.pred_is_v = a.hot_pred_is_v; p1.op = a.p.op; p1.thr = a.p.dval;
    p1.nrows = nrows;
    p1.out_entries = e1; p1.out_counts = c1; p1.out_cap = cap1;
    int lg1 = 0;
    while ((1 << lg1) < np1) lg1++;
    p1.nparts = np1; p1.shift = 32 - lg1; p1.flags = flags;
    p1.debug = (int)env_i64("VNM_PART_DEBUG", 0);
    p1.spill = spill; p1.spill_cap = spill_cap;
    p1.nval = h->plan.n_cols;
    p1.has_vmask = a.part_vmask;
    if (wide) {
        for (int c = 0; c < h->plan.n_cols; c++) p1.vcols[c] = a.cols[c];
        p1.wp = a.p;
        p1.wpred = a.pred;
    }
    auto pring_cap = [&](int np) -> int { int cap = (int)((size_t)128 * 1024 / 16 / (size_t)np); cap = std::min(cap, 64) / 16 * 16; return cap; };
    auto pring_lds = [&](int np) -> size_t { return (size_t)np * pring_cap(np) * 16; };
    const bool ring_ok = !wide && !a.has_expr && !h->pring_off && env_i64("VNM_PART_RING", 7) != 0 && (a.keys[0].offset & 1) == 0 && (!h->plan.n_cols || (a.cols[0].offset & 1) == 0) &&
                         (!h->pred_set || a.hot_pred_is_v || (a.pred.offset & 1) == 0) && h->plan.n_cols > 0;
    const bool ring1 = ring_ok && np1 <= 256 && np1 >= 128 && (env_i64("VNM_PART_RING", 7) & 1);
    const bool ring2 = ring_ok && levels == 2 && np2 <= 256 && np2 >= 128 && (env_i64("VNM_PART_RING", 7) & 2);
    const bool ring2_512 = ring_ok && levels == 2 && np2 == 512 && (env_i64("VNM_PART_RING", 7) & 4);
    {
        KernelTimer timer("agg_part_scatter1", s);
        if (ring1) VNM_TRY(pick_bool(p1.has_pred && !p1.pred_is_v, [&](auto pv) { return launch_dyn(pring_scatter_kernel<true, 2, 16, decltype(pv)::value>, grid1, PT_BLOCK, pring_lds(np1), s, p1, pring_cap(np1)); }));
        else if (!wide) part_scatter_kernel<true><<<grid1, PT_BLOCK, 0, s>>>(p1);
        else VNM_TRY((pick_int<1, 7>(E, [&](auto e) { return launch_dyn(part_scatter_wide_kernel<true, decltype(e)::value, pw_items(decltype(e)::value)>, grid1, PT_BLOCK, (size_t)pw_tile(E) * ebytes, s, p1); })));
    }
    VNM_HIP(hipGetLastError());
    auto overflowed = [&]() -> int {
        unsigned long long f = 0;
        if (hipMemcpyAsync(&f, flags, 8, hipMemcpyDeviceToHost, s) != hipSuccess || hipStreamSynchronize(s) != hipSuccess) return -1;
        return f ? 1 : 0;
    };
    {
        int ov = overflowed();
        if (ov > 0 && ring1) {
            h->pring_off = true;
            route_note("hash_partitions:rings_failed", "a region overflowed or a sub-tile needed too many rounds: the tile-sorting scatter takes the batch and every later one");
            pool.done(e1); pool.done(c1); pool.done(flags); pool.done(spill);
            return partitioned_aggregate(h, a, nrows, s, spill_out, n_spill_out);
        }
        if (ov) return ov < 0 ? set_error("aggregate: partition pass failed") : 2;
    }
    if (ring1) route_note("hash_partitions:rings", "%d x %d partitions: (key, value) entries through LDS rings, whole 256-byte blocks out", np1, np2);

    const ulonglong2* fin_e = e1;
    const uint32_t* fin_c = c1;
    int64_t fin_cap = cap1, nfinal = np1;
    int fin_regions = grid1;
    ulonglong2* e2 = nullptr;
    uint32_t* c2 = nullptr;
    if (levels == 2) {
        const int64_t per_pg = (int64_t)grid1 * rows_per_wg / np1 / split2;
        const int64_t cap2 = per_pg / np2 + (int64_t)((double)(per_pg / np2) * std::max(0.25, slack)) + 256;
        e2 = (ulonglong2*)pool.take((size_t)np1 * np2 * split2 * cap2 * ebytes);
        c2 = (uint32_t*)pool.take((size_t)np1 * np2 * split2 * 4);
        if (!e2 || !c2) return 1;
        PartArgs p2{};
        p2.in_entries = e1; p2.in_counts = c1; p2.in_cap = cap1; p2.in_regions = grid1; p2.in_split = split2;
        p2.out_entries = e2; p2.out_counts = c2; p2.out_cap = cap2;
        p2.nparts = np2; p2.shift = 15; p2.flags = flags;
        p2.debug = p1.debug;
        p2.spill = spill; p2.spill_cap = spill_cap;
        p2.nval = h->plan.n_cols;
        p2.has_vmask = a.part_vmask;
        {
            KernelTimer timer("agg_part_scatter2", s);
            const int g2 = np1 * p2.in_split;
            if (ring2) VNM_TRY(launch_dyn(pring_scatter_kernel<false, 2, 16, false>, g2, PT_BLOCK, pring_lds(np2), s, p2, pring_cap(np2)));
            else if (ring2_512) VNM_TRY(launch_dyn(pring_scatter_kernel<false, 1, 8, false>, g2, PT_BLOCK, (size_t)512 * 16 * 16, s, p2, 16));
            else if (!wide) part_scatter_kernel<false><<<g2, PT_BLOCK, 0, s>>>(p2);
            else VNM_TRY((pick_int<1, 7>(E, [&](auto e) {
                constexpr int EW = decltype(e)::value;
                if constexpr (EW <= 2) { if (np2 < 128) return launch_dyn(part_scatter_wide_kernel<false, EW, 4>, g2, PT_BLOCK, (size_t)PT_BLOCK * 4 * ebytes, s, p2); }
                return launch_dyn(part_scatter_wide_kernel<false, EW, pw_items(EW)>, g2, PT_BLOCK, (size_t)PT_BLOCK * pw_items(EW) * ebytes, s, p2);
            })));
        }
        VNM_HIP(hipGetLastError());
        {
            int ov = overflowed();
            if (ov > 0 && (ring2 || ring2_512)) {
                h->pring_off = true;
                route_note("hash_partitions:rings_failed", "level 2: a region overflowed or a sub-tile needed too many rounds: the tile-sorting scatter takes the batch and every later one");
                pool.done(e1); pool.done(c1); pool.done(e2); pool.done(c2); pool.done(flags); pool.done(spill);
                return partitioned_aggregate(h, a, nrows, s, spill_out, n_spill_out);
            }
            if (ov) return ov < 0 ? set_error("aggregate: partition pass failed") : 2;
        }
        fin_e = e2; fin_c = c2; fin_cap = cap2; nfinal = (int64_t)np1 * np2; fin_regions = p2.in_split;
    }

    int splits = 1;
    if (nfinal < (int64_t)cus * 4) {
        splits = (int)std::min<int64_t>(256, ((int64_t)cus * 8 + nfinal - 1) / nfinal);
        if (splits > fin_regions) splits = fin_regions;
    }
    const bool to_table = splits > 1 && !(h->have_table || h->have_run);
    const bool dup_run = splits > 1 && !to_table;
    const int64_t dstride = to_table ? 2 : std::min<int64_t>(nrows, (h->hint * 2 + (1 << 20)) * (dup_run ? splits : 1)) + 2;
    uint64_t* rk = (uint64_t*)pool.take((size_t)dstride * 8 * 2);
    uint64_t* ra = (uint64_t*)pool.take((size_t)dstride * 8 * h->plan.n_words);
    if (!rk || !ra) return 1;
    unsigned long long* dir = nullptr;
    if (!to_table && !dup_run) {
        dir = (unsigned long long*)pool.take((size_t)nfinal * 16);
        if (!dir) return 1;
// ... 330 lines not shown
        if constexpr (TB >= 9) return launch_resident(dpart_final_kernel<uint16_t, TB, false, OUT, float>, df.nfinal, blk, 0, occ_max, s, df);
        break;
    }
    return set_error("aggregate: no dense final pass of form %d for tables of 2^%d slots (internal error)", form, TB);
}
int launch_dense_final(const DFinalArgs& df, int tb, int out, bool lo64, hipStream_t s, bool exact = false, const DSet* only_set = nullptr) {
    KernelTimer timer("agg_part_final", s);
    int form = DFF_PLAIN, tbk = tb;
    if (df.fx_q != 0.0 && only_set && !only_set->pad && only_set->regions > 0 && only_set->regions <= 512 && tb >= 7 && tb <= 13 &&
        (!df.has_side || (out != DF_TABLE && env_i64("VNM_DFX_LEAN_SIDE", 1))) && env_i64("VNM_DFX_LEAN", 1)) form = DFF_LEAN;
    else if (df.fx_q == 0.0 && lo64) {
        if (tb < 9 || tb > 12) return set_error("aggregate: no 64-bit compensation variant for this table size (internal error)");
        form = DFF_LO64;
    } else if (df.fx_q != 0.0) {
        if (tb < 7 || tb > 13) return set_error("aggregate: fixed-point entries with this table size (internal error)");
        form = DFF_FIXED;
    } else if (exact && (tb == 12 || tb == 13) && out != DF_TABLE) form = DFF_EXACT;
    else if (tb < 9 || tb > 12) tbk = 13;
    VNM_TRY((pick_int<7, 13>(tbk, [&](auto tbc) {
        return pick_out(out, [&](auto outc) { return launch_dense_final_as<decltype(tbc)::value, decltype(outc)::value>(form, df, only_set, s); });
    })));
    VNM_HIP(hipGetLastError());
    return 0;
}

int upload_segs(vnm_agg* h, int64_t tile, const VSeg** dev, int* nseg, int64_t* ntiles, PoolScope& pool, hipStream_t s) {
    const std::vector<vnm_agg::QBatch>& q = *h->segs_active;
    h->seg_host.resize(q.size());
    int64_t t = 0;
    for (size_t i = 0; i < q.size(); i++) {
        VSeg& g = h->seg_host[i];
        g.kp = (const uint64_t*)q[i].key.values + q[i].key.offset;
        g.vp = (const uint64_t*)q[i].col.values + q[i].col.offset;
        g.pp = h->pred_set ? (const double*)q[i].pred.values + q[i].pred.offset : nullptr;
        g.vvalid = nullptr; g.voff = 0;
        g.nrows = q[i].nrows;
        g.first_tile = t;
        t += (q[i].nrows + tile - 1) / tile;
    }
    VSeg* d = (VSeg*)pool.take(q.size() * sizeof(VSeg));
    if (!d) return 1;
    VNM_HIP(hipMemcpyAsync(d, h->seg_host.data(), q.size() * sizeof(VSeg), hipMemcpyHostToDevice, s));
    *dev = d; *nseg = (int)q.size(); *ntiles = t;
    return 0;
}

int complete_pending(vnm_agg* h, hipStream_t s, int out = DF_RUN, const DFinalArgs* cols = nullptr, int64_t* n_out = nullptr) {
    DensePending* pd = h->pending;
    if (!pd) return 0;
    if (out == DF_RUN && h->have_run) VNM_TRY(merge_run_into_table(h, s));
    DFinalArgs df = pd->df;
    PoolScope pool;
    uint64_t* rk = nullptr; uint64_t* ra = nullptr;
    if (out == DF_RUN) {
        rk = (uint64_t*)pool.take((size_t)pd->dstride * 8 * 2);
        ra = (uint64_t*)pool.take((size_t)pd->dstride * 8 * h->plan.n_words);
        if (!rk || !ra) return 1;
        df.dkey = rk; df.dacc = ra;
    } else if (out == DF_COLS) {
        df.n_out = cols->n_out;
        for (int c = 0; c < cols->n_out; c++) { df.out_kind[c] = cols->out_kind[c]; df.out_ptr[c] = cols->out_ptr[c]; df.key_field[c] = cols->key_field[c]; }
        df.pack_n = cols->pack_n;
        for (int j = 0; j < cols->pack_n; j++) { df.pack_shift[j] = cols->pack_shift[j]; df.pack_bits[j] = cols->pack_bits[j]; df.pack_lo[j] = cols->pack_lo[j]; }
        if (cols->has_side) { df.has_side = 1; df.side = cols->side; df.side_bloom = cols->side_bloom; df.side_bloom_mask = cols->side_bloom_mask; df.side_found = cols->side_found; }
    } else {
        if (!pd->table) pd->table = (DTabSlot*)pool_alloc(sizeof(DTabSlot) << df.map.bits);
        if (!pd->table) return 1;
        df.table = pd->table;
    }
    df.dstride = (out == DF_COLS && cols->dstride > 0) ? cols->dstride : pd->dstride;
    pool_free(pd->dsets);
    pd->dsets = (DSet*)pool_alloc(pd->sets.size() * sizeof(DSet));
    if (!pd->dsets) return 1;
    VNM_HIP(hipMemcpyAsync(pd->dsets, pd->sets.data(), pd->sets.size() * sizeof(DSet), hipMemcpyHostToDevice, s));
    df.sets = pd->dsets; df.nsets = (int)pd->sets.size();
    unsigned long long fl[5] = {0, 0, 0, 0, 0};
    uint64_t* psum = nullptr; float* plo = nullptr; uint32_t* pcnt = nullptr;
    if (pd->fsplits > 1 && df.has_side) return set_error("aggregate: side table with a split final pass (internal error)");
    if (pd->fsplits > 1) {
        const size_t cells = (size_t)pd->nfinal * pd->fsplits << pd->tb;
        psum = (uint64_t*)pool.take(cells * 8); plo = (float*)pool.take(cells * 4); pcnt = (uint32_t*)pool.take(cells * 4);
        if (!psum || !plo || !pcnt) return 1;
    }
    for (int attempt = 0; attempt < 2; attempt++) {
        VNM_HIP(hipMemsetAsync(df.flags, 0, 16, s));
        if (attempt == 0 && pd->fsplits > 1) {
            DFinalArgs ds = df;
            ds.splits = pd->fsplits; ds.part_sum = psum; ds.part_lo = plo; ds.part_cnt = pcnt;
            const int cus = device_info().num_cus;
            KernelTimer timer("agg_part_final", s);
            const int g3 = (int)std::min<int64_t>(pd->nfinal * pd->fsplits, (int64_t)cus * 8);
            if (pd->tb == 9) dpart_final_kernel<uint16_t, 9, true><<<g3, 512, 0, s>>>(ds);
            else if (pd->tb == 10) dpart_final_kernel<uint16_t, 10, true><<<g3, 512, 0, s>>>(ds);
            else if (pd->tb == 11) dpart_final_kernel<uint16_t, 11, true><<<g3, 512, 0, s>>>(ds);
            else if (pd->tb == 12) dpart_final_kernel<uint16_t, 12, true><<<g3, VNM_DF12_BLOCK, 0, s>>>(ds);
            else dpart_final_kernel<uint16_t, 13, true><<<g3, 1024, 0, s>>>(ds);
            if (out != DF_COLS) ds.n_out = 0;
            dpart_merge_kernel<<<(int)(pd->nfinal << (pd->tb - 9)), 512, 0, s>>>(ds, pd->tb);
            VNM_HIP(hipGetLastError());
        } else if (attempt == 1 && pd->tb == 13 && df.fx_q == 0.0) {
            df.sub_bits = 1;
            for (int sub = 0; sub < 2; sub++) { df.sub = sub; VNM_TRY(launch_dense_final(df, 12, out, true, s)); }
        } else {
            if (df.has_side) {
                VNM_HIP(hipMemsetAsync(df.side_found, 0, (size_t)df.side.cap + 2, s));
                VNM_HIP(hipMemsetAsync(df.flags + 4, 0, 8, s));
            }
            const int xmode = (int)env_i64("VNM_DF_EXACT", 1);
            const bool exact = attempt == 0 && df.w_sum >= 0 && df.w_lo >= 0 && !df.sub_bits && (xmode == 2 || (xmode == 1 && pd->exact_ok()));
            if (exact) route_note("dense:exact_adds", "2^%d-slot tables without compensation words: %lld rows, values below 2^%d with lowest bits >= 2^%d",
                                  pd->tb, (long long)pd->rows, (int)pd->x_exp - 1022, (int)(0xFFFFu - pd->x_inv) - 1075);
            VNM_TRY(launch_dense_final(df, pd->tb, out, attempt == 1, s, exact, pd->sets.size() == 1 ? &pd->sets[0] : nullptr));
            if (df.has_side) {
                KernelTimer timer("agg_side_append", s);
                dside_append_kernel<<<(int)std::min<int64_t>(((int64_t)df.side.cap + 2 + 255) / 256, (int64_t)device_info().num_cus * 8), 256, 0, s>>>(df, 0);
                dside_append_kernel<<<1, 256, 0, s>>>(df, 1);
                VNM_HIP(hipGetLastError());
            }
        }
        VNM_HIP(hipMemcpyAsync(fl, df.flags, 40, hipMemcpyDeviceToHost, s));
        VNM_HIP(hipStreamSynchronize(s));
        if (!fl[0]) break;
        if (out == DF_TABLE) return 2;
        if (attempt == 1) return set_error("aggregate: dense final pass failed (internal error)");
    }
    if (getenv("VNM_AGG_TRACE")) fprintf(stderr, "[agg] dense final (deferred, %zu batch%s): mode %d -> groups %llu\n", pd->sets.size(),
                                         pd->sets.size() == 1 ? "" : "es", out, fl[1]);
    if (n_out) *n_out = (int64_t)fl[1];
    if (out == DF_COLS && cols->null_pos) *cols->null_pos = df.has_side ? (int64_t)fl[4] : 0;
    if (out == DF_RUN) {
        pool.keep(rk); pool.keep(ra);
        h->run_key = rk; h->run_acc = ra; h->run_stride = pd->dstride; h->run_n = (int64_t)fl[1];
        h->run_dir = nullptr; h->run_nfin = 0;
        h->have_run = true;
        delete pd;
        h->pending = nullptr;
    }
    return 0;
}


struct DensePlan {
    bool generic, has_val;
    bool vn, vn_lists;
    bool fx_base;
    int tb, pbits, levels;
    int p1, p2, np1, np2;
    int64_t nfinal;
    int fsplits;
    bool count8;
    int c8_cb, c8_sub;
    bool fx;
    double fx_q;
    bool w32, w32_1;
    int grid1, split2;
    int64_t cap1, cap2;
    bool c16_1;
    int pmajor;
    int64_t spill_cap, nspill_cap, dstride;
    int rcap1, rcap2;
    bool ring_limit;
    int ring_pairs1, ring_pairs2;
};
constexpr int DENSE_REDO = 4;

int plan_dense_entries(const vnm_agg* h, const AggArgs& a, bool generic, const DGenArgs& g, bool vn_fold, bool null_lists, DensePlan* p) {
    p->generic = generic;
    p->has_val = generic ? g.has_val != 0 : true;
    if ((h->segs_active || h->kn_valid) && generic) return 2;
    if (h->kn_valid && h->segs_active) return 2;
    p->vn = p->has_val && a.cols[0].validity != nullptr && (generic || vn_fold);
    if (p->vn && ((!vn_fold && !null_lists) || a.has_expr)) return 2;
    if (vn_fold && (generic || !a.hot_pred_is_v)) return 2;
    p->vn_lists = p->vn && !vn_fold;
    p->fx_base = !generic && p->has_val && (!p->vn || vn_fold) && !a.has_expr && !(h->kn_valid && p->vn) && a.hot_comp && a.hot_w_sum >= 0 &&
                 env_i64("VNM_DENSE_DEFER", 1) && env_i64("VNM_DENSE_FX", 1) && a.cols[0].type == VNM_F64 && (env_i64("VNM_DENSE_RING", 3) & 3) == 3;
    return 0;
}

int sample_fixed_point(vnm_agg* h, const AggArgs& a, int64_t nrows, hipStream_t s) {
    h->fx_state = -1;
    PoolScope pool;
    unsigned long long* d = (unsigned long long*)pool.take(64);
    if (!d) return 1;
    unsigned long long got = 0;
    VNM_HIP(hipMemsetAsync(d, 0, 8, s));
    const int64_t srows = h->segs_active ? (*h->segs_active)[0].nrows : nrows;
    const int64_t m = std::min<int64_t>(srows, 1 << 16);
    fx_sample_kernel<<<(int)std::min<int64_t>((m + 255) / 256, 256), 256, 0, s>>>((const double*)a.cols[0].values + a.cols[0].offset, srows, m, d);
    VNM_HIP(hipGetLastError());
    VNM_HIP(hipMemcpyAsync(&got, d, 8, hipMemcpyDeviceToHost, s));
    VNM_HIP(hipStreamSynchronize(s));
    const uint32_t xinv = (uint32_t)got, xexp = (uint32_t)(got >> 32);
    if (xinv == 0 && xexp == 0) { h->fx_state = 1; h->fx_qe = -16; }
    else if (xexp < 2047) {
        const int L = (int)(0xFFFFu - xinv) - 1075, E = (int)xexp - 1022;
        const bool narrow = E - L <= 16 && env_i64("VNM_DENSE_FX_NARROW", 1) != 0;
        const int room = narrow ? 18 : 31;
        const int spare = room - (E - L);
        if (spare >= 0) {
            int qe = L - spare / 2;
            if (qe > 0) qe = 0;
            if (qe >= -1000 && E - qe <= room) { h->fx_state = 1; h->fx_qe = qe; h->fx_narrow = narrow; }
        }
    }
    if (getenv("VNM_AGG_TRACE")) fprintf(stderr, "[agg] fixed-point entries: sample says %s (qe %d)\n", h->fx_state == 1 ? "yes" : "no", h->fx_qe);
    return 0;
}

int plan_dense_geometry(const vnm_agg* h, const AggArgs& a, int64_t nrows, const DGenArgs& g, DensePlan* p) {
    const int cus = device_info().num_cus;
    const DenseMap& mp = h->dmap;
    const bool generic = p->generic, has_val = p->has_val;
    const bool fx_ok = p->fx_base && h->fx_state == 1;
    int tb = (int)env_i64("VNM_DENSE_TBITS", 12);
    tb = std::max(DP_TBITS_MIN, std::min(DP_TBITS_MAX, tb));
    while (tb > DP_TBITS_MIN && mp.bits - tb < 11) tb--;
    while (tb < DP_TBITS_MAX && mp.bits - tb > 18) tb++;
    const int one_level_bits = DP_TBITS_MAX + (has_val && env_i64("VNM_DENSE_ONE_LEVEL_512", 0) == 0 ? 8 : 9);
    if (mp.bits <= one_level_bits && env_i64("VNM_DENSE_ONE_LEVEL", 1)) tb = std::max(DP_TBITS_MIN, std::min(DP_TBITS_MAX, mp.bits - (int)env_i64("VNM_DENSE_ONE_P", 8)));
    if (mp.bits < 20) tb = (int)env_i64("VNM_DENSE_SMALL_TBITS", 11);
    if (mp.bits - tb < 5 && env_i64("VNM_DENSE_MIN_PARTS32", 1)) tb = std::max(9, mp.bits - 5);
    if (fx_ok && mp.bits >= 20 && mp.bits <= 22 && env_i64("VNM_DENSE_FX_ONE_LEVEL", 1)) tb = mp.bits - 9;
    const bool fx_small = fx_ok && mp.bits >= (int)env_i64("VNM_DENSE_FX_SMALL_MIN_BITS", 15) && mp.bits <= 19 && env_i64("VNM_DENSE_FX_SMALL", 1) != 0;
    if (fx_small) tb = std::max(7, mp.bits - 9);
    if (generic) {
        int tmax = DP_TBITS_MAX;
        while (tmax > 9 && ((size_t)dgen_slot_bytes(g) << tmax) > 64 * 1024) tmax--;
        if (mp.bits - tmax == 9 && tmax < DP_TBITS_MAX && ((size_t)dgen_slot_bytes(g) << (tmax + 1)) <= (size_t)env_i64("VNM_DGEN_BIG_LDS_KB", 128) * 1024) tmax++;
        if (((size_t)dgen_slot_bytes(g) << tmax) > 128 * 1024) return 2;
        if (tb > tmax) tb = tmax;
        if (mp.bits - tb > 18) return 2;
    }
    p->c8_cb = h->count_cb ? h->count_cb : ((h->hint == 0 || nrows <= 64 * h->hint) ? 8 : (nrows <= 16384 * h->hint ? 16 : 0));
    const int c8_tmax = p->c8_cb == 8 ? DC8_BITS : DC8_BITS - 1;
    p->count8 = generic && !has_val && g.n_lds == 0 && !p->vn && !h->count8_off && h->heavy_share == 0.0 && p->c8_cb != 0 && mp.bits >= DP_TBITS_MAX + 10 &&
                mp.bits <= c8_tmax + 9 + 1 && env_i64("VNM_DENSE_COUNT8", 1);
    p->c8_sub = p->count8 ? std::max(0, mp.bits - c8_tmax - 9) : 0;
    if (p->count8) tb = mp.bits - 9 - p->c8_sub;
    p->tb = tb;
    p->pbits = p->count8 ? 9 : mp.bits - tb;
    p->levels = p->pbits > 9 ? 2 : 1;
    const int pbits = p->pbits, levels = p->levels;
    p->nfinal = (int64_t)1 << pbits;
    int p1 = levels == 2 ? (int)env_i64("VNM_DENSE_P1", fx_ok ? (pbits + 1) / 2 : pbits / 2) : pbits;
    if (levels == 2) { if (p1 > 9) p1 = 9; if (pbits - p1 > 9) p1 = pbits - 9; }
    p->p1 = p1; p->p2 = pbits - p1;
    p->np1 = 1 << p1; p->np2 = levels == 2 ? 1 << p->p2 : 0;
    const int np1 = p->np1, np2 = p->np2;
    const int64_t tile1 = PT_TILE;
    const int grid1 = (int)std::min<int64_t>((int64_t)cus * env_i64("VNM_DENSE_GRID1_PER_CU", 2), (nrows + tile1 - 1) / tile1);
    int split2 = std::max(2, (grid1 + PT_MAX_REGIONS - 1) / PT_MAX_REGIONS);
    split2 = std::max(split2, std::min(grid1, (cus * 2 + np1 - 1) / np1));
    if (h->heavy_share > 0.0) split2 = std::min(grid1, split2 * (int)env_i64("VNM_DENSE_SKEW_SPLIT", 8));
    p->grid1 = grid1; p->split2 = split2;
    const int64_t tiles_per_wg = ((nrows + tile1 - 1) / tile1 + grid1 - 1) / grid1;
    const int64_t rows_per_wg = tiles_per_wg * tile1;
    int64_t cap1 = ((rows_per_wg / np1 + rows_per_wg / np1 / 5 + 512) + 15) & ~15LL;
    const bool odd_cap = env_i64("VNM_DENSE_ODD_CAP", 1) != 0;
    if (odd_cap && ((cap1 / 16) & 1) == 0) cap1 += 16;
    if (fx_ok && h->fx_narrow && levels == 1) { cap1 = (cap1 + 31) & ~31LL; if (((cap1 / 32) & 1) == 0) cap1 += 32; }
    p->cap1 = cap1;
    p->c16_1 = levels == 1 && !p->count8;
    int fsplits = 1;
    if (levels == 1 && !p->count8 && ((int64_t)1 << pbits) < (int64_t)cus * 2) {
        fsplits = (int)std::min<int64_t>(grid1, ((int64_t)cus * env_i64("VNM_DENSE_SPLIT_WGS", 4) + ((int64_t)1 << pbits) - 1) >> pbits);
        if (fsplits < 2) fsplits = 1;
    }
    if (fx_small && levels == 1) fsplits = 1;
    p->fsplits = fsplits;
    p->fx = fx_ok && fsplits == 1 && !p->count8 && tb >= (fx_small ? 7 : 11) && tb <= 13;
    p->fx_q = p->fx ? std::ldexp(1.0, h->fx_qe) : 0.0;
    p->w32 = p->fx && h->fx_narrow;
    p->w32_1 = p->w32 && levels == 1;
    if (levels == 2) {
        const int64_t per_pg = (int64_t)grid1 * rows_per_wg / np1 / split2;
        int64_t cap2 = ((per_pg / np2 + per_pg / np2 / 4 + 256) + 15) & ~15LL;
        if (odd_cap && ((cap2 / 16) & 1) == 0) cap2 += 16;
        if (p->w32) { cap2 = (cap2 + 31) & ~31LL; if (((cap2 / 32) & 1) == 0) cap2 += 32; }
        p->cap2 = cap2;
    }
    p->spill_cap = nrows / 2 + (1 << 20);
    p->nspill_cap = p->vn_lists ? nrows / 4 + (1 << 20) : 0;
    p->dstride = std::min<int64_t>(h->dense_span, nrows) + 2;
    p->pmajor = (int)env_i64("VNM_DENSE_PRODUCER_MAJOR", 0);
    const int use_ring = (int)env_i64("VNM_DENSE_RING", 3);
    p->ring_limit = env_i64("VNM_DENSE_RING_LIMIT", 1) != 0;
    p->rcap1 = p->w32_1 ? ring_cap_w32(np1) : ((use_ring & 1) && !a.has_expr ? ring_cap_for(np1, p->fx ? 8 : (has_val ? 8 : 0) + (p->c16_1 ? 2 : 4)) : 0);
    if (levels == 2) p->rcap2 = p->fx ? (p->w32 ? ring_cap_w32(np2) : ring_cap_for(np2, 8)) : ((use_ring & 2) ? ring_cap_for(np2, (has_val ? 8 : 0) + 2) : 0);
    p->ring_pairs1 = (int)env_i64("VNM_DENSE_RING_PAIRS", 4);
    if (p->fx && levels == 2 && getenv("VNM_DENSE_RING_PAIRS") == nullptr) p->ring_pairs1 = 2;
    p->ring_pairs2 = levels == 2 ? (int)env_i64("VNM_DENSE_RING_PAIRS2", p->fx && p->w32 ? 4 : 2) : 0;
    return 0;
}

struct DenseBuffers {
    PoolScope pool;
    unsigned long long* flags = nullptr;
    double* v1 = nullptr; void* c1 = nullptr; uint32_t* n1 = nullptr;
    double* v2 = nullptr; void* c2 = nullptr; uint32_t* n2 = nullptr;
    ulonglong2* spill = nullptr;
    uint64_t* nspill = nullptr;
    uint64_t* rk = nullptr; uint64_t* ra = nullptr;
    template <class T> void take(T*& p, size_t bytes) { p = (T*)pool.take(bytes); }
    void free_all() { while (pool.n > 0) pool.done(pool.blocks[pool.n - 1]); }
};

int dense_allocate(const DensePlan& p, DenseBuffers& b, hipStream_t s) {
    b.take(b.flags, 128);
    b.take(b.v1, p.has_val ? (size_t)p.np1 * p.grid1 * p.cap1 * (p.w32_1 ? 4 : 8) : 8);
    b.take(b.c1, p.fx ? 16 : (size_t)p.np1 * p.grid1 * p.cap1 * (p.c16_1 ? 2 : 4));
    b.take(b.n1, (size_t)p.np1 * p.grid1 * 4);
    b.take(b.spill, (size_t)p.spill_cap * 16);
    if (p.vn_lists) b.take(b.nspill, (size_t)p.nspill_cap * 8);
    if (!b.flags || !b.v1 || !b.c1 || !b.n1 || !b.spill || (p.vn_lists && !b.nspill)) return 1;
    VNM_HIP(hipMemsetAsync(b.flags, 0, 128, s));
    fill_u64_kernel<<<1, 1, 0, s>>>((uint64_t*)b.flags + 11, F64_NEG_ZERO, 1);
    VNM_HIP(hipGetLastError());
    return 0;
}

int fold_null_rows(const vnm_agg* h, const AggArgs& a, const unsigned long long* flags, hipStream_t s) {
    if (!h->kn_valid) return 0;
    const GTable& gt = h->g;
    const uint64_t slot = gt.cap + 1;
    dnull_fold_kernel<<<1, 64, 0, s>>>(flags + 8, gt.tag + slot,
                                       a.hot_w_rows >= 0 ? gt.acc + (uint64_t)a.hot_w_rows * gt.stride + slot : nullptr,
                                       a.hot_w_valid >= 0 ? gt.acc + (uint64_t)a.hot_w_valid * gt.stride + slot : nullptr,
                                       a.hot_w_sum >= 0 ? gt.acc + (uint64_t)a.hot_w_sum * gt.stride + slot : nullptr,
                                       a.hot_comp && a.hot_w_sum >= 0 ? (int64_t)gt.stride : 0);
    VNM_HIP(hipGetLastError());
    return 0;
}

int dense_scatter1_launch(vnm_agg* h, const DensePlan& p, DenseBuffers& b, DPartArgs& d1, hipStream_t s) {
    const bool pv = d1.has_pred && !d1.pred_is_v;
    if (!p.rcap1)
        return pick_bool(p.c16_1, [&](auto c16) {
            using CT = std::conditional_t<decltype(c16)::value, uint16_t, uint32_t>;
            if (p.vn) { dpart_scatter_kernel<true, CT, true, true><<<p.grid1, PT_BLOCK, 0, s>>>(d1); return 0; }
            return pick_bool(p.has_val, [&](auto hv) { dpart_scatter_kernel<true, CT, decltype(hv)::value><<<p.grid1, PT_BLOCK, 0, s>>>(d1); return 0; });
        });
    const bool plain_val = p.has_val && !p.vn;
    const RingLaunch r{p.grid1, p.rcap1, ring_sub_tile_pairs(p.ring_pairs1, pv, p.ring_limit, p.np1, p.rcap1, p.w32_1), p.ring_limit,
                       plain_val && h->segs_active != nullptr, plain_val && h->kn_valid != nullptr, s};
    if (r.seg && !r.kn && upload_segs(h, (int64_t)2 * r.pairs * 1024, &d1.segs, &d1.nseg, &d1.nsub, b.pool, s)) return 1;
    if (p.fx && p.vn)
        return pick_bool(p.w32_1, [&](auto w32) { return ring_scatter<true, uint32_t, true, false, true, true, decltype(w32)::value>(r, d1); });
    if (p.fx)
        return pick_bool(p.w32_1, [&](auto w32) {
            return pick_bool(pv, [&](auto pvc) { return ring_scatter<true, uint32_t, true, decltype(pvc)::value, false, true, decltype(w32)::value>(r, d1); });
        });
    return pick_bool(p.c16_1, [&](auto c16) {
        using CT = std::conditional_t<decltype(c16)::value, uint16_t, uint32_t>;
        return pick_bool(pv, [&](auto pvc) {
            if (p.vn) return ring_scatter<true, CT, true, decltype(pvc)::value, true>(r, d1);
            return pick_bool(p.has_val, [&](auto hv) { return ring_scatter<true, CT, decltype(hv)::value, decltype(pvc)::value, false>(r, d1); });
        });
    });
}

int dense_scatter1(vnm_agg* h, const AggArgs& a, int64_t nrows, const DensePlan& p, DenseBuffers& b, DPartArgs& d1, hipStream_t s) {
    d1.map = h->dmap;
    d1.kp = (const uint64_t*)a.keys[0].values + a.keys[0].offset;
    d1.vp = p.has_val ? (const double*)a.cols[0].values + a.cols[0].offset : nullptr;
    d1.has_expr = a.has_expr; d1.expr = a.expr;
    d1.pp = h->pred_set ? (const double*)a.pred.values + a.pred.offset : nullptr;
    d1.has_pred = h->pred_set; d1.pred_is_v = a.hot_pred_is_v; d1.op = a.p.op; d1.thr = a.p.dval;
    d1.nrows = nrows;
    d1.out_vals = b.v1; d1.out_codes = b.c1; d1.out_counts = b.n1; d1.out_cap = p.cap1;
    d1.nparts = p.np1; d1.out_bits = h->dmap.bits - p.p1;
    d1.producer_major = p.pmajor;
    d1.nt_store = (int)env_i64("VNM_DENSE_NT", p.levels == 2 && p.np2 >= 256 ? 1 : 0) & 1;
    d1.ready_list = (int)env_i64("VNM_DENSE_READY_LIST", 1) & 1;
    d1.flags = b.flags; d1.spill = b.spill; d1.spill_cap = p.spill_cap;
    d1.fx_q = p.fx_q; d1.fx_inv_q = p.fx ? std::ldexp(1.0, -h->fx_qe) : 0.0;
    d1.fx_lim = p.w32 ? (1LL << 18) - 1 : 2147483647LL;
    if (p.vn) { d1.vvalid = a.cols[0].validity; d1.voff = a.cols[0].offset; d1.nspill = b.nspill; d1.nspill_cap = p.nspill_cap; }
    if (h->kn_valid) {
        if (ensure_table(h, 1024, s, true)) return 1;
        uint64_t* scr = (uint64_t*)(b.flags + 8);
        d1.kvalid = h->kn_valid; d1.koff = h->kn_off;
        d1.nk_tag = scr;
        d1.nk_rows = a.hot_w_rows >= 0 ? scr + 1 : nullptr;
        d1.nk_valid = a.hot_w_valid >= 0 ? scr + 2 : nullptr;
        d1.nk_sum = a.hot_w_sum >= 0 ? scr + 3 : nullptr;
        d1.nk_lo_stride = a.hot_comp && a.hot_w_sum >= 0 ? 1 : 0;
    }
    {
        KernelTimer timer("agg_part_scatter1", s);
        VNM_TRY(dense_scatter1_launch(h, p, b, d1, s));
    }
    VNM_HIP(hipGetLastError());
    return 0;
}

int dense_scatter2(const vnm_agg* h, const DensePlan& p, DenseBuffers& b, const DPartArgs& d1, hipStream_t s) {
    b.take(b.v2, p.has_val ? (size_t)p.np1 * p.np2 * p.split2 * p.cap2 * (p.w32 ? 4 : 8) : 8);
    b.take(b.c2, p.fx ? 16 : (size_t)p.np1 * p.np2 * p.split2 * p.cap2 * 2);
    b.take(b.n2, (size_t)p.np1 * p.np2 * p.split2 * 4);
    if (!b.v2 || !b.c2 || !b.n2) return 1;
    DPartArgs d2{};
    d2.map = h->dmap;
    d2.in_vals = b.v1; d2.in_codes = (const uint32_t*)b.c1; d2.in_counts = b.n1; d2.in_cap = p.cap1;
    d2.in_regions = p.grid1; d2.in_split = p.split2; d2.in_bits = h->dmap.bits - p.p1;
    d2.in_pstride = p.pmajor ? 1 : p.grid1; d2.in_rstride = p.pmajor ? p.np1 : 1;
    d2.out_vals = b.v2; d2.out_codes = b.c2; d2.out_counts = b.n2; d2.out_cap = p.cap2;
    d2.nparts = p.np2; d2.out_bits = p.tb;
    d2.flags = b.flags; d2.spill = b.spill; d2.spill_cap = p.spill_cap;
    d2.nspill = b.nspill; d2.nspill_cap = p.nspill_cap;
    d2.nt_store = ((int)env_i64("VNM_DENSE_NT", 0) >> 1) & 1;
    d2.ready_list = ((int)env_i64("VNM_DENSE_READY_LIST", 1) >> 1) & 1;
    d2.fx_q = d1.fx_q; d2.fx_inv_q = d1.fx_inv_q; d2.fx_lim = d1.fx_lim;
    const int grid2 = p.np1 * p.split2;
    const RingLaunch r{grid2, p.rcap2, ring_sub_tile_pairs(p.ring_pairs2, false, p.ring_limit, p.np2, p.rcap2, p.w32), p.ring_limit, false, false, s};
    {
        KernelTimer timer("agg_part_scatter2", s);
        if (p.fx) VNM_TRY(pick_bool(p.w32, [&](auto w32) { return ring_scatter<false, uint32_t, true, false, false, true, decltype(w32)::value>(r, d2); }));
        else if (p.rcap2) VNM_TRY(pick_bool(p.has_val, [&](auto hv) { return ring_scatter<false, uint16_t, decltype(hv)::value, false, false>(r, d2); }));
        else VNM_TRY(pick_bool(p.has_val, [&](auto hv) { dpart_scatter_kernel<false, uint16_t, decltype(hv)::value><<<grid2, PT_BLOCK, 0, s>>>(d2); return 0; }));
    }
    VNM_HIP(hipGetLastError());
    return 0;
}

int dense_final_count8(vnm_agg* h, const DensePlan& p, const DenseBuffers& b, DGenArgs& g, hipStream_t s) {
    for (int cb = p.c8_cb;;) {
        const int tbc = std::min(p.tb, cb == 8 ? DC8_BITS : DC8_BITS - 1), subc = p.c8_sub + (p.tb - tbc);
        g.tbits = tbc;
        const size_t lds = ((size_t)1 << tbc) * (size_t)(cb / 8);
        {
            KernelTimer timer("agg_part_final", s);
            VNM_TRY(launch_resident(cb == 8 ? dcount8_final_kernel<8> : dcount8_final_kernel<16>, p.nfinal << subc, 1024, lds, 2, s, g, subc));
        }
        VNM_HIP(hipGetLastError());
        if (cb == 16) break;
        unsigned long long f6[6];
        VNM_HIP(hipMemcpyAsync(f6, b.flags, sizeof(f6), hipMemcpyDeviceToHost, s));
        VNM_HIP(hipStreamSynchronize(s));
        if (!(f6[0] && f6[5])) break;
        cb = 16;
        h->count_cb = 16;
        VNM_HIP(hipMemsetAsync(b.flags, 0, 16, s));
        VNM_HIP(hipMemsetAsync(b.flags + 5, 0, 8, s));
    }
    return 0;
}

int dense_final_generic(const DensePlan& p, DenseBuffers& b, DGenArgs& g, hipStream_t s) {
    const size_t slots = (size_t)1 << p.tb;
    const size_t lds = slots * dgen_slot_bytes(g);
    if (p.fsplits > 1) {
        const size_t work = (size_t)p.nfinal * p.fsplits;
        g.part_w = (uint64_t*)b.pool.take(std::max<size_t>(8, work * g.n_lds * slots * 8));
        g.part_cnt = (uint32_t*)b.pool.take(work * slots * 4);
        if (!g.part_w || !g.part_cnt) return 1;
        g.splits = p.fsplits;
    }
    KernelTimer timer("agg_part_final", s);
    VNM_TRY(pick_bool(p.has_val, [&](auto hv) {
        return pick_bool(p.fsplits > 1, [&](auto sp) {
            return launch_resident(dgen_final_kernel<decltype(hv)::value, decltype(sp)::value>, p.nfinal * (decltype(sp)::value ? p.fsplits : 1), 512, lds, 8, s, g);
        });
    }));
    if (p.fsplits > 1) dgen_merge_kernel<<<(int)(p.nfinal << (p.tb - 9)), 512, 0, s>>>(g);
    return 0;
}

int dense_final_split(const DensePlan& p, DenseBuffers& b, DFinalArgs& df, hipStream_t s) {
    const size_t cells = (size_t)p.nfinal * p.fsplits << p.tb;
    df.part_sum = (uint64_t*)b.pool.take(cells * 8); df.part_lo = (float*)b.pool.take(cells * 4); df.part_cnt = (uint32_t*)b.pool.take(cells * 4);
    if (!df.part_sum || !df.part_lo || !df.part_cnt) return 1;
    df.splits = p.fsplits;
    KernelTimer timer("agg_part_final", s);
    VNM_TRY((pick_int<9, 13>(p.tb >= 9 && p.tb <= 12 ? p.tb : 13, [&](auto tbc) {
        constexpr int TB = decltype(tbc)::value;
        return launch_resident(dpart_final_kernel<uint16_t, TB, true>, p.nfinal * p.fsplits, TB >= 13 ? 1024 : (TB == 12 ? VNM_DF12_BLOCK : 512), 0, 8, s, df);
    })));
    dpart_merge_kernel<<<(int)(p.nfinal << (p.tb - 9)), 512, 0, s>>>(df, p.tb);
    return 0;
}

int dense_defer_final(vnm_agg* h, const AggArgs& a, int64_t nrows, const DensePlan& p, DenseBuffers& b, const DSet& fin, DFinalArgs& df, hipStream_t s,
                      ulonglong2** spill_out, int64_t* n_spill_out) {
    const DenseMap& mp = h->dmap;
    unsigned long long fl0[8];
    VNM_HIP(hipMemcpyAsync(fl0, b.flags, 64, hipMemcpyDeviceToHost, s));
    VNM_HIP(hipStreamSynchronize(s));
    route_note(h->kn_valid ? "dense:nullable_key" : (h->segs_active ? "dense:stream_segments" : (p.vn ? "dense:nullable_value" : (p.levels == 1 && p.p1 == 5 && p.tb <= 10 ? "dense:32_partitions" :
               (p.fsplits > 1 ? "dense:split_final" : (p.levels == 2 ? "dense:two_levels" : "dense:one_level"))))),
               "2^%d codes, 2^%d-slot final tables, p1 %d p2 %d, final pass deferred%s: %s", mp.bits, p.tb, p.p1, p.p2, p.vn ? ", nullable value" : "", fl0[0] || (p.fx && fl0[7]) ? "scatter FAILED (the batch goes another way)" : "ok");
    if (getenv("VNM_AGG_TRACE"))
        fprintf(stderr, "[agg] dense: bits %d tb %d levels %d p1 %d p2 %d -> scatter fail %llu spilled %llu, final pass deferred (bound %lld)\n",
                mp.bits, p.tb, p.levels, p.p1, p.p2, fl0[0], fl0[2], (long long)p.dstride);
    if (p.fx && fl0[7]) {
        if (h->fx_narrow) {
            h->fx_narrow = false;
            h->fx_qe = std::max(h->fx_qe - 6, -1000);
            route_note("dense:fixed_point_misfit", "a value outside 2^%d * [-2^18, 2^18): the batch is redone with 64-bit entry words", h->fx_qe + 6);
            return DENSE_REDO;
        }
        h->fx_state = -1;
        route_note("dense:fixed_point_misfit", "a value outside 2^%d * [-2^31, 2^31): the batch is redone with float64 entries", h->fx_qe);
        return DENSE_REDO;
    }
    if (fl0[0]) return 2;
    if (p.fx) route_note("dense:fixed_point", "%s entry words, quantum 2^%d", p.w32 ? (p.levels == 1 ? "4-byte" : "8-byte, then 4-byte") : "8-byte", h->fx_qe);
    if (fold_null_rows(h, a, b.flags, s)) return 1;
    b.pool.done(b.rk); b.pool.done(b.ra);
    if (fl0[2]) { b.pool.keep(b.spill); *spill_out = b.spill; *n_spill_out = (int64_t)fl0[2]; }
    else { *spill_out = nullptr; *n_spill_out = 0; }
    if ((int64_t)fl0[2] > nrows / 16) h->dense_state = -1;
    DensePending* pd = h->pending;
    const int64_t pending_max_rows = std::min<int64_t>(env_i64("VNM_DENSE_PENDING_MAX_ROWS", 3LL << 29), (1LL << 32) - 1);
    if (pd && (pd->tb != p.tb || pd->levels != p.levels || pd->p1 != p.p1 || pd->fsplits != p.fsplits || pd->sets.size() >= DP_MAX_SETS ||
               pd->rows + nrows > pending_max_rows || pd->df.fx_q != p.fx_q || pd->df.fx_w32 != (p.w32 ? 1 : 0) || memcmp(&pd->df.map, &mp, sizeof(DenseMap)) != 0)) {
        VNM_TRY(complete_pending(h, s));
        pd = nullptr;
    }
    if (!pd) {
        pd = new DensePending();
        df.dkey = nullptr; df.dacc = nullptr;
        pd->df = df; pd->tb = p.tb; pd->levels = p.levels; pd->p1 = p.p1; pd->fsplits = p.fsplits; pd->nfinal = p.nfinal; pd->dstride = 0;
        b.pool.keep(b.flags); pd->blocks.push_back(b.flags);
        h->pending = pd;
    }
    pd->dstride = std::min<int64_t>(h->dense_span, pd->dstride + nrows) + 2;
    pd->rows += nrows;
    if (p.rcap1 && p.has_val && !a.has_expr && !p.fx) { pd->x_inv = std::max(pd->x_inv, (uint32_t)fl0[6]); pd->x_exp = std::max(pd->x_exp, (uint32_t)(fl0[6] >> 32)); }
    else pd->x_known = false;
    pd->sets.push_back(fin);
    void* const held[3] = {p.levels == 2 ? (void*)b.v2 : (void*)b.v1, p.levels == 2 ? b.c2 : b.c1, p.levels == 2 ? (void*)b.n2 : (void*)b.n1};
    for (void* blk : held) { b.pool.keep(blk); pd->blocks.push_back(blk); }
    return 0;
}

int dense_hand_over(vnm_agg* h, const AggArgs& a, int64_t nrows, const DensePlan& p, DenseBuffers& b, hipStream_t s, ulonglong2** spill_out, int64_t* n_spill_out,
                    uint64_t** nspill_out, int64_t* n_nspill_out) {
    VNM_HIP(hipGetLastError());
    unsigned long long fl[4];
    VNM_HIP(hipMemcpyAsync(fl, b.flags, 32, hipMemcpyDeviceToHost, s));
    VNM_HIP(hipStreamSynchronize(s));
    if (!fl[0]) {
        if (fold_null_rows(h, a, b.flags, s)) return 1;
        VNM_HIP(hipStreamSynchronize(s));
    }
    route_note(p.count8 ? "dense:count_bytes" : p.generic ? (p.fsplits > 1 ? "dense:generic_split_final" : "dense:generic") : (p.vn ? "dense:nullable_value" : (p.fsplits > 1 ? "dense:split_final" : "dense:run")),
               "2^%d codes, 2^%d-slot final tables, levels %d, p1 %d p2 %d, %d final splits: %s", h->dmap.bits, p.tb, p.levels, p.p1, p.p2, p.fsplits, fl[0] ? "FAILED (the batch goes another way)" : "ok");
    if (getenv("VNM_AGG_TRACE"))
        fprintf(stderr, "[agg] dense%s%s: bits %d tb %d levels %d p1 %d p2 %d splits %d -> fail %llu groups %llu spilled %llu + %llu NULL-value rows (dstride %lld)\n",
                p.generic ? " generic" : "", p.vn ? " nullable" : "", h->dmap.bits, p.tb, p.levels, p.p1, p.p2, p.fsplits, fl[0], fl[1], fl[2], fl[3], (long long)p.dstride);
    if (fl[0]) {
        if (!p.count8) return 2;
        h->count8_off = true;
        return DENSE_REDO;
    }
    if (fl[2]) { b.pool.keep(b.spill); *spill_out = b.spill; *n_spill_out = (int64_t)fl[2]; }
    else { *spill_out = nullptr; *n_spill_out = 0; }
    if (p.vn && fl[3]) { b.pool.keep(b.nspill); *nspill_out = b.nspill; *n_nspill_out = (int64_t)fl[3]; }
    if ((int64_t)(fl[2] + fl[3]) > nrows / 16) h->dense_state = -1;
    b.pool.keep(b.rk); b.pool.keep(b.ra);
    h->run_key = b.rk; h->run_acc = b.ra; h->run_stride = p.dstride; h->run_n = (int64_t)fl[1];
    h->run_dir = nullptr; h->run_nfin = 0;
    h->have_run = true;
    return 0;
}

int dense_partitioned_aggregate(vnm_agg* h, const AggArgs& a, int64_t nrows, hipStream_t s, ulonglong2** spill_out, int64_t* n_spill_out,
                                bool generic = false, uint64_t** nspill_out = nullptr, int64_t* n_nspill_out = nullptr, bool vn_fold = false) {
    DGenArgs g{};
    if (generic && !dgen_program(h, a, &g)) return 2;
    DensePlan p{};
    VNM_TRY(plan_dense_entries(h, a, generic, g, vn_fold, nspill_out != nullptr, &p));
    if (nspill_out) { *nspill_out = nullptr; *n_nspill_out = 0; }
    if (p.fx_base && h->fx_state == 0) VNM_TRY(sample_fixed_point(h, a, nrows, s));
    VNM_TRY(plan_dense_geometry(h, a, nrows, g, &p));
    DenseBuffers b;
    auto redo = [&]() { b.free_all(); return dense_partitioned_aggregate(h, a, nrows, s, spill_out, n_spill_out, generic, nspill_out, n_nspill_out, vn_fold); };
    VNM_TRY(dense_allocate(p, b, s));
    if (p.fx && (!p.rcap1 || (p.levels == 2 && !p.rcap2))) { h->fx_state = -1; return redo(); }
    if ((h->segs_active || h->kn_valid) && (!p.rcap1 || p.vn)) return 2;
    DPartArgs d1{};
    VNM_TRY(dense_scatter1(h, a, nrows, p, b, d1, s));
    if (p.levels == 2) VNM_TRY(dense_scatter2(h, p, b, d1, s));
    DSet fin{b.v1, b.c1, b.n1, p.cap1, p.grid1, 1, p.grid1, 0};
    if (p.levels == 2) fin = DSet{b.v2, b.c2, b.n2, p.cap2, p.split2, 1, p.split2, 0};
    else if (p.pmajor) { fin.pstride = 1; fin.rstride = p.np1; }
    fin.pad = fin.cap < 2048 ? 1 : 0;
    b.take(b.rk, (size_t)p.dstride * 8 * 2);
    b.take(b.ra, (size_t)p.dstride * 8 * h->plan.n_words);
    if (!b.rk || !b.ra) return 1;
    DFinalArgs df{};
    df.map = h->dmap;
    df.vals = fin.vals; df.codes = fin.codes; df.counts = fin.counts; df.cap = fin.cap; df.regions = fin.regions; df.nfinal = p.nfinal;
    df.pstride = fin.pstride; df.rstride = fin.rstride;
    df.w_rows = a.hot_w_rows; df.w_valid = a.hot_w_valid; df.w_sum = a.hot_w_sum;
    df.w_lo = a.hot_comp && a.hot_w_sum >= 0 ? a.hot_w_sum + 1 : -1;
    df.dkey = b.rk; df.dacc = b.ra; df.dstride = p.dstride; df.flags = b.flags;
    df.fx_q = p.fx_q; df.fx_w32 = p.w32 ? 1 : 0;
    const bool own_run = generic || !env_i64("VNM_DENSE_DEFER", 1);
    if (own_run && h->pending) {
        int rc = complete_pending(h, s);
        if (!rc) rc = merge_run_into_table(h, s);
        if (rc) return 1;
    }
    if (generic) {
        g.map = h->dmap; g.tbits = p.tb;
        g.pstride = fin.pstride; g.rstride = fin.rstride;
        g.vals = p.count8 ? nullptr : fin.vals; g.codes = fin.codes; g.counts = fin.counts; g.cap = fin.cap; g.regions = fin.regions; g.nfinal = p.nfinal;
        g.dkey = b.rk; g.dacc = b.ra; g.dstride = p.dstride; g.flags = b.flags;
    }
    if (p.count8) VNM_TRY(dense_final_count8(h, p, b, g, s));
    else if (generic) VNM_TRY(dense_final_generic(p, b, g, s));
    else if (p.fsplits > 1 && own_run) VNM_TRY(dense_final_split(p, b, df, s));
    else if (env_i64("VNM_DENSE_DEFER", 1)) {
        const int rc = dense_defer_final(h, a, nrows, p, b, fin, df, s, spill_out, n_spill_out);
        return rc == DENSE_REDO ? redo() : rc;
    } else VNM_TRY(launch_dense_final(df, p.tb, DF_RUN, false, s));
    const int rc = dense_hand_over(h, a, nrows, p, b, s, spill_out, n_spill_out, nspill_out, n_nspill_out);
    return rc == DENSE_REDO ? redo() : rc;
}


int dense_two_aggregate(vnm_agg* h, const AggArgs& a, int64_t nrows, hipStream_t s) {
    const int cus = device_info().num_cus;
    const DenseMap& mp = h->dmap;
    int tb = 11;
    if (mp.bits - tb > 15) tb = 12;
    const int pbits = mp.bits - tb;
    if (pbits > 15 || pbits < 10 || a.has_expr) return 2;
    const int p2 = std::min(8, (pbits + 1) / 2), p1 = pbits - p2;
    if (p1 > 7 || p1 < 5) return 2;
    const int np1 = 1 << p1, np2 = 1 << p2;
    const int64_t tile1 = PT_TILE;
    const int grid1 = (int)std::min<int64_t>((int64_t)cus * 2, (nrows + tile1 - 1) / tile1);
    int split2 = std::max(2, (grid1 + PT_MAX_REGIONS - 1) / PT_MAX_REGIONS);
    split2 = std::max(split2, std::min(grid1, (cus * 2 + np1 - 1) / np1));
    const int64_t tiles_per_wg = ((nrows + tile1 - 1) / tile1 + grid1 - 1) / grid1;
    const int64_t rows_per_wg = tiles_per_wg * tile1;
    int64_t cap1 = ((rows_per_wg / np1 + rows_per_wg / np1 / 5 + 512) + 15) & ~15LL;
    if (((cap1 / 16) & 1) == 0) cap1 += 16;
    const int64_t per_pg = (int64_t)grid1 * rows_per_wg / np1 / split2;
    int64_t cap2 = ((per_pg / np2 + per_pg / np2 / 4 + 256) + 15) & ~15LL;
    if (((cap2 / 16) & 1) == 0) cap2 += 16;
    const int64_t nfinal = (int64_t)1 << pbits;
    const int64_t dstride = std::min<int64_t>(h->dense_span, nrows) + 2;
    PoolScope pool;
    unsigned long long* flags = (unsigned long long*)pool.take(64);
    double* v1 = (double*)pool.take((size_t)np1 * grid1 * cap1 * 8);
    double* w1 = (double*)pool.take((size_t)np1 * grid1 * cap1 * 8);
    uint32_t* c1 = (uint32_t*)pool.take((size_t)np1 * grid1 * cap1 * 4);
    uint32_t* n1 = (uint32_t*)pool.take((size_t)np1 * grid1 * 4);
    double* v2 = (double*)pool.take((size_t)np1 * np2 * split2 * cap2 * 8);
    double* w2 = (double*)pool.take((size_t)np1 * np2 * split2 * cap2 * 8);
    uint16_t* c2 = (uint16_t*)pool.take((size_t)np1 * np2 * split2 * cap2 * 2);
    uint32_t* n2 = (uint32_t*)pool.take((size_t)np1 * np2 * split2 * 4);
    uint64_t* rk = (uint64_t*)pool.take((size_t)dstride * 8 * 2);
    uint64_t* ra = (uint64_t*)pool.take((size_t)dstride * 8 * h->plan.n_words);
    if (!flags || !v1 || !w1 || !c1 || !n1 || !v2 || !w2 || !c2 || !n2 || !rk || !ra) return 1;
    VNM_HIP(hipMemsetAsync(flags, 0, 64, s));
// ... 70 lines not shown
```

Measured before the change: 154.5 billion rows/s.

## Write 4-byte biased fixed-point words from the first dense scatter level

Result: faster. 160.9 billion rows/s (median of 6 runs) (+4.1%).

```diff
diff --git a/vinum_amd/csrc/vnm_agg.hip b/vinum_amd/csrc/vnm_agg.hip
--- a/vinum_amd/csrc/vnm_agg.hip
+++ b/vinum_amd/csrc/vnm_agg.hip
@@ -373,6 +373,9 @@
     bool pack_null_seen = false;
     bool pring_off = false;
     bool fx_narrow = false;
+    bool fx_narrow1 = true, fx_ranged = false;
+    int fx_low = 0;
+    double fx_smin = 0.0, fx_smax = 0.0;
     int fxn_state = 0, fxn_qe[3] = {0, 0, 0};
     bool null_inputs_seen = false;
     bool count8_off = false;
diff --git a/vinum_amd/csrc/vnm_agg_dense.inc b/vinum_amd/csrc/vnm_agg_dense.inc
--- a/vinum_amd/csrc/vnm_agg_dense.inc
+++ b/vinum_amd/csrc/vnm_agg_dense.inc
@@ -65,6 +65,9 @@
     int64_t nspill_cap;
     double fx_q, fx_inv_q;
     int64_t fx_lim;
+    int64_t fx_bias;
+    int fx_biased;
+    int64_t fx_dlo, fx_dhi;
 };
 constexpr uint32_t DP_NULL32 = 0x80000000u;
 __device__ __forceinline__ bool fx_encode(double v, double inv_q, int64_t* m, int64_t lim = 2147483647LL) {
@@ -336,6 +339,8 @@
 constexpr int DR_FB = 16;
 typedef double dr_v2 __attribute__((ext_vector_type(2)));
 typedef uint32_t dr_u2 __attribute__((ext_vector_type(2)));
+template <bool FROM_ROWS, typename CT, bool FX>
+constexpr bool ring_reads_w32() { return FX && !FROM_ROWS && sizeof(CT) == 4; }
 template <bool FROM_ROWS, typename CT, bool HAS_VAL, int DR_BLOCK, int DR_PAIRS, bool PV = false, bool VN = false, int MAXR = 0, bool SEG = false, bool KN = false,
           bool V2 = false, bool FX = false, bool W32 = false>
 __global__ __launch_bounds__(DR_BLOCK) void dring_scatter_kernel(DPartArgs a, int ring_cap) {
@@ -344,10 +349,14 @@
     static_assert(!W32 || FX, "32-bit entry words are fixed-point words");
     constexpr int FB = W32 ? 32 : DR_FB, EPL = FB / 8;
     constexpr int NE = 2 * DR_PAIRS;
+    constexpr bool IN32 = ring_reads_w32<FROM_ROWS, CT, FX>();
+    static_assert(!IN32 || (W32 && DR_PAIRS >= 2), "32-bit words in: 32-bit words out, whole quads per lane");
+    using RT = std::conditional_t<FX, uint32_t, CT>;
+    const bool wbiased = FROM_ROWS && W32 && a.fx_biased != 0;
     const int np = a.nparts;
     double* const rv = (double*)dr_lds;
     double* const rv2 = rv + (V2 ? (size_t)np * ring_cap : 0);
-    CT* const rc = (CT*)(dr_lds + (HAS_VAL ? (size_t)np * ring_cap * (V2 ? 2 : 1) : 0));
+    RT* const rc = (RT*)(dr_lds + (HAS_VAL ? (size_t)np * ring_cap * (V2 ? 2 : 1) : 0));
     __shared__ uint32_t fill[PT_MAXP], head[PT_MAXP], cursor[PT_MAXP];
     __shared__ uint32_t s_retry[2];
     __shared__ uint32_t s_nready[2];
@@ -374,7 +383,7 @@
     }
     double* const ov = a.out_vals;
     double* const ov2 = a.out_vals2;
-    CT* const oc = (CT*)a.out_codes;
+    RT* const oc = (RT*)a.out_codes;
     const uint32_t ocap = (uint32_t)a.out_cap;
 
     auto insert = [&](uint32_t c, double v, double w2) -> bool {
@@ -394,12 +403,26 @@
         }
         if (HAS_VAL) rv[(size_t)p * ring_cap + slot] = v;
         if (V2) rv2[(size_t)p * ring_cap + slot] = w2;
-        rc[(size_t)p * ring_cap + slot] = dense_rem<CT>(c, remmask);
+        rc[(size_t)p * ring_cap + slot] = dense_rem<RT>(c, remmask);
         return true;
     };
     auto fx_rem = [&](size_t li) -> uint32_t { return W32 ? ((const uint32_t*)rv)[li] & remmask : (uint32_t)(((const uint64_t*)rv)[li] & (uint64_t)remmask); };
     auto fx_val = [&](size_t li) -> double {
-        return W32 ? (double)((int32_t)((const uint32_t*)rv)[li] >> a.out_bits) * a.fx_q : (double)((int64_t)((const uint64_t*)rv)[li] >> a.out_bits) * a.fx_q;
+        if (W32) {
+            const uint32_t w = ((const uint32_t*)rv)[li];
+            return (double)(wbiased ? (int64_t)(w >> a.out_bits) + a.fx_bias : (int64_t)((int32_t)w >> a.out_bits)) * a.fx_q;
+        }
+        return (double)((int64_t)((const uint64_t*)rv)[li] >> a.out_bits) * a.fx_q;
+    };
+    auto fx_slot = [&](double val, double* slot) -> uint32_t {
+        int64_t m;
+        if (!fx_encode(val, a.fx_inv_q, &m, a.fx_lim)) return wbiased ? 3u : 1u;
+        if (wbiased) {
+            m -= a.fx_bias;
+            if ((uint64_t)m >> (32 - a.out_bits)) return m < a.fx_dlo || m > a.fx_dhi ? 3u : 1u;
+        }
+        *slot = fx_bits(m);
+        return 0;
     };
     auto flush = [&](bool drain) {
         const int j = tid & 7;
@@ -434,7 +457,7 @@
                             if (a.nt_store) __builtin_nontemporal_store(x2, (dr_v2*)(ov2 + at)); else *(dr_v2*)(ov2 + at) = x2;
                         }
                         if (FX) {
-                        } else if (sizeof(CT) == 4) {
+                        } else if (sizeof(RT) == 4) {
                             const dr_u2 y = *(const dr_u2*)(rc + li);
                             if (a.nt_store) __builtin_nontemporal_store(y, (dr_u2*)(oc + at)); else *(dr_u2*)(oc + at) = y;
                         } else {
@@ -455,15 +478,15 @@
                     const unsigned long long pos = base + (unsigned long long)__popcll(m & ((1ULL << (lane - j)) - 1ULL)) * FB + EPL * j;
                     if ((int64_t)(pos + EPL) <= a.spill_cap) {
                         for (int e = 0; e < EPL; e++)
-                            a.spill[pos + e] = make_ulonglong2(dense_key_of(a.map, prefix | (p << a.out_bits) | (FX ? fx_rem(li + e) : dense_rem_code<CT>(rc[FX ? 0 : li + e]))),
+                            a.spill[pos + e] = make_ulonglong2(dense_key_of(a.map, prefix | (p << a.out_bits) | (FX ? fx_rem(li + e) : dense_rem_code<RT>(rc[FX ? 0 : li + e]))),
                                                                (unsigned long long)__double_as_longlong(FX ? fx_val(li + e) : (HAS_VAL ? rv[li + e] : 0.0)));
                     } else __hip_atomic_store(&a.flags[0], 1ULL, __ATOMIC_RELAXED, __HIP_MEMORY_SCOPE_AGENT);
                 } else {
                     for (int e = 0; e < EPL; e++)
                         if ((uint32_t)(EPL * j + e) < n_here) {
                             if (FX) dense_spill(a, dense_key_of(a.map, prefix | (p << a.out_bits) | fx_rem(li + e)), fx_val(li + e));
-                            else dense_spill(a, dense_key_of(a.map, prefix | (p << a.out_bits) | dense_rem_code<CT>(rc[FX ? 0 : li + e])), HAS_VAL ? rv[li + e] : 0.0,
-                                             dense_rem_null<CT>(rc[FX ? 0 : li + e]));
+                            else dense_spill(a, dense_key_of(a.map, prefix | (p << a.out_bits) | dense_rem_code<RT>(rc[FX ? 0 : li + e])), HAS_VAL ? rv[li + e] : 0.0,
+                                             dense_rem_null<RT>(rc[FX ? 0 : li + e]));
                         }
                 }
                 done += n_here;
@@ -516,7 +539,7 @@
                         const unsigned long long pos = base + at++;
                         if ((int64_t)pos < a.spill_cap)
                             a.spill[pos] = make_ulonglong2(dense_key_of(a.map, prefix | c[e]),
-                                                           (unsigned long long)__double_as_longlong(FX ? (double)fx_of(v[e]) * a.fx_q : (HAS_VAL ? v[e] : 0.0)));
+                                                           (unsigned long long)__double_as_longlong(FX ? (double)(fx_of(v[e]) + (wbiased ? a.fx_bias : 0)) * a.fx_q : (HAS_VAL ? v[e] : 0.0)));
                         else __hip_atomic_store(&a.flags[0], 1ULL, __ATOMIC_RELAXED, __HIP_MEMORY_SCOPE_AGENT);
                     }
                 }
@@ -534,7 +557,7 @@
     uint32_t nk_cnt = 0;
     constexpr bool XT = FROM_ROWS && HAS_VAL && !V2 && !FX;
     uint32_t xinv = 0, xexp = 0;
-    bool fx_bad = false;
+    bool fx_wide = false; bool fx_bad = false;
     if (FROM_ROWS && !SEG) {
         const int64_t sub = (int64_t)NE * DR_BLOCK;
         const int64_t nsub = (a.nrows + sub - 1) / sub;
@@ -600,7 +623,7 @@
                 }
                 c[e] = (((uint32_t)d * a.map.mul) & a.map.mask) | (VN && isnull ? DP_NULL32 : 0u);
                 v[e] = VN && isnull ? 0.0 : val;
-                if (FX) { int64_t m; if (!fx_encode(val, a.fx_inv_q, &m, a.fx_lim)) { fx_bad = true; continue; } v[e] = fx_bits(m); }
+                if (FX) { const uint32_t miss = fx_slot(val, &v[e]); if (miss) { fx_bad = true; if (W32) fx_wide |= miss > 1u; continue; } }
                 if (V2) w2[V2 ? e : 0] = val2;
                 if (XT) exact_track(v[e], xinv, xexp);
                 okmask |= 1u << e;
@@ -666,7 +689,7 @@
                 if (d > (uint64_t)a.map.mask) { dense_spill(a, key, val, isnull); continue; }
                 c[e] = (((uint32_t)d * a.map.mul) & a.map.mask) | (VN && isnull ? DP_NULL32 : 0u);
                 v[e] = VN && isnull ? 0.0 : val;
-                if (FX) { int64_t m; if (!fx_encode(val, a.fx_inv_q, &m, a.fx_lim)) { fx_bad = true; continue; } v[e] = fx_bits(m); }
+                if (FX) { const uint32_t miss = fx_slot(val, &v[e]); if (miss) { fx_bad = true; if (W32) fx_wide |= miss > 1u; continue; } }
                 if (XT) exact_track(v[e], xinv, xexp);
                 okmask |= 1u << e;
             }
@@ -676,6 +699,7 @@
             cur = nxt;
         }
     } else {
+        constexpr int EPU = IN32 ? 4 : 2, NU = NE / EPU;
         __shared__ uint32_t rstart[PT_MAX_REGIONS + 1];
         const int pin = blockIdx.x / a.in_split;
         const int per_max = (a.in_regions + a.in_split - 1) / a.in_split;
@@ -685,39 +709,52 @@
         const int64_t region0 = (int64_t)pin * a.in_pstride + (int64_t)first * a.in_rstride;
         if (tid == 0) {
             uint32_t run = 0;
-            for (int rj = 0; rj < per; rj++) { rstart[rj] = run; run += (a.in_counts[region0 + rj * a.in_rstride] + 1) / 2; }
+            for (int rj = 0; rj < per; rj++) { rstart[rj] = run; run += (a.in_counts[region0 + rj * a.in_rstride] + EPU - 1) / EPU; }
             rstart[per] = run;
         }
         __syncthreads();
         const uint32_t total_in = rstart[per];
-        double2 ev[DR_PAIRS], ev2[V2 ? DR_PAIRS : 1];
-        uint2 ec[DR_PAIRS];
+        double2 ev[NU], ev2[V2 ? NU : 1];
+        uint2 ec[NU];
         uint32_t okm = 0;
         int reg = 0;
-        auto load_pairs = [&](uint32_t t0) {
+        auto load_units = [&](uint32_t t0) {
             okm = 0;
 #pragma unroll
-            for (int u = 0; u < DR_PAIRS; u++) {
+            for (int u = 0; u < NU; u++) {
                 const uint32_t v = t0 + (uint32_t)u * DR_BLOCK + tid;
                 if (v < total_in) {
                     int lo = reg;
                     while (rstart[lo + 1] <= v) lo++;
                     reg = lo;
-                    const uint32_t e0 = 2u * (v - rstart[lo]);
+                    const uint32_t e0 = (uint32_t)EPU * (v - rstart[lo]);
                     const int64_t rg = region0 + lo * a.in_rstride;
                     const int64_t at = rg * a.in_cap + e0;
-                    if (HAS_VAL) ev[u] = *(const double2*)(a.in_vals + at);
+                    if (IN32) ev[u] = *(const double2*)((const uint32_t*)a.in_vals + at);
+                    else if (HAS_VAL) ev[u] = *(const double2*)(a.in_vals + at);
                     if (V2) ev2[V2 ? u : 0] = *(const double2*)(a.in_vals2 + at);
                     if (!FX) ec[u] = *(const uint2*)(a.in_codes + at);
-                    okm |= (e0 + 1 < a.in_counts[rg] ? 3u : 1u) << (2 * u);
+                    const uint32_t left = a.in_counts[rg] - e0;
+                    okm |= (left >= (uint32_t)EPU ? (1u << EPU) - 1u : (1u << left) - 1u) << (EPU * u);
                 }
             }
         };
-        load_pairs(0);
-        for (uint32_t t0 = 0; t0 < total_in; t0 += DR_PAIRS * DR_BLOCK) {
+        load_units(0);
+        for (uint32_t t0 = 0; t0 < total_in; t0 += NU * DR_BLOCK) {
             uint32_t c[NE]; double v[NE]; double w2[V2 ? NE : 1];
 #pragma unroll
-            for (int u = 0; u < DR_PAIRS; u++) {
+            for (int u = 0; u < NU; u++) {
+                if constexpr (IN32) {
+                    const uint64_t w01 = (uint64_t)__double_as_longlong(ev[u].x), w23 = (uint64_t)__double_as_longlong(ev[u].y);
+                    const uint32_t w[4] = {(uint32_t)w01, (uint32_t)(w01 >> 32), (uint32_t)w23, (uint32_t)(w23 >> 32)};
+                    const uint32_t inmask = (1u << a.in_bits) - 1u;
+#pragma unroll
+                    for (int k = 0; k < 4; k++) {
+                        c[4 * u + k] = w[k] & inmask;
+                        v[4 * u + k] = fx_bits((int64_t)(w[k] >> a.in_bits) + a.fx_bias);
+                    }
+                    continue;
+                }
                 if (FX) {
                     const uint64_t w0 = (uint64_t)__double_as_longlong(ev[u].x), w1 = (uint64_t)__double_as_longlong(ev[u].y);
                     const uint64_t inmask = ((uint64_t)1 << a.in_bits) - 1;
@@ -730,14 +767,17 @@
                 if (V2) { w2[V2 ? 2 * u : 0] = ev2[V2 ? u : 0].x; w2[V2 ? 2 * u + 1 : 0] = ev2[V2 ? u : 0].y; }
             }
             const uint32_t okmask = okm;
-            load_pairs(t0 + DR_PAIRS * DR_BLOCK);
+            load_units(t0 + NU * DR_BLOCK);
             rounds(c, v, w2, okmask);
         }
     }
     flush(true);
     __syncthreads();
     if (tid < np) a.out_counts[out_base + (int64_t)tid * out_stride] = cursor[tid];
-    if (FX && FROM_ROWS) { if (__syncthreads_or(fx_bad ? 1 : 0) && tid == 0) __hip_atomic_store(&a.flags[7], 1ULL, __ATOMIC_RELAXED, __HIP_MEMORY_SCOPE_AGENT); }
+    if (FX && FROM_ROWS) {
+        const int wider = W32 ? __syncthreads_or(fx_wide ? 1 : 0) : 0;
+        if (__syncthreads_or(fx_bad ? 1 : 0) && tid == 0) __hip_atomic_fetch_or(&a.flags[7], wider ? 3ULL : 1ULL, __ATOMIC_RELAXED, __HIP_MEMORY_SCOPE_AGENT);
+    }
     if (XT) {
         if (tid < 2) s_spill[tid] = 0;
         __syncthreads();
@@ -2127,17 +2167,40 @@
     }
 }
 
-__global__ __launch_bounds__(256) void fx_sample_kernel(const double* vals, int64_t nrows, int64_t m, unsigned long long* out) {
+struct FxSampleRange {
+    unsigned long long* out;
+    const double* pp;
+    int has_pred, op;
+    double thr;
+    const uint8_t* vvalid;
+    int64_t voff;
+};
+__global__ __launch_bounds__(256) void fx_sample_kernel(const double* vals, int64_t nrows, int64_t m, unsigned long long* out, FxSampleRange r) {
     __shared__ uint32_t sx[2];
-    if (threadIdx.x < 2) sx[threadIdx.x] = 0;
+    __shared__ unsigned long long sr[2];
+    if (threadIdx.x < 2) { sx[threadIdx.x] = 0; sr[threadIdx.x] = 0; }
     __syncthreads();
     const int64_t stride = (int64_t)gridDim.x * blockDim.x;
     uint32_t xinv = 0, xexp = 0;
-    for (int64_t i = (int64_t)blockIdx.x * blockDim.x + threadIdx.x; i < m; i += stride) exact_track(vals[(int64_t)(((__int128)i * nrows) / m)], xinv, xexp);
+    uint64_t nmin = 0, xmax = 0;
+    for (int64_t i = (int64_t)blockIdx.x * blockDim.x + threadIdx.x; i < m; i += stride) {
+        const int64_t row = (int64_t)(((__int128)i * nrows) / m);
+        const double v = vals[row];
+        exact_track(v, xinv, xexp);
+        if (!r.out || v != v) continue;
+        if (r.vvalid && !((r.vvalid[(r.voff + row) >> 3] >> ((r.voff + row) & 7)) & 1)) continue;
+        if (r.has_pred && !cmp_apply<double>(r.op, r.pp ? r.pp[row] : v, r.thr)) continue;
+        const uint64_t e = enc_f64(v);
+        nmin = ~e > nmin ? ~e : nmin;
+        xmax = e > xmax ? e : xmax;
+    }
     if (xinv) atomicMax(&sx[0], xinv);
     if (xexp) atomicMax(&sx[1], xexp);
+    if (nmin) atomicMax(&sr[0], (unsigned long long)nmin);
+    if (xmax) atomicMax(&sr[1], (unsigned long long)xmax);
     __syncthreads();
     if (threadIdx.x < 2 && sx[threadIdx.x]) atomicMax((uint32_t*)out + threadIdx.x, sx[threadIdx.x]);
+    if (threadIdx.x < 2 && r.out && sr[threadIdx.x]) atomicMax(&r.out[threadIdx.x], sr[threadIdx.x]);
 }
 
 __global__ __launch_bounds__(256) void dense_sample_range_kernel(const uint64_t* keys, int64_t nrows, int64_t m, uint64_t sign,
diff --git a/vinum_amd/csrc/vnm_agg_fxn.inc b/vinum_amd/csrc/vnm_agg_fxn.inc
--- a/vinum_amd/csrc/vnm_agg_fxn.inc
+++ b/vinum_amd/csrc/vnm_agg_fxn.inc
@@ -418,7 +418,7 @@
         const int64_t srows = q ? (*q)[0].nrows : nrows;
         const int64_t m = std::min<int64_t>(srows, 1 << 16);
         for (int c = 0; c < NV; c++)
-            fx_sample_kernel<<<(int)std::min<int64_t>((m + 255) / 256, 256), 256, 0, s>>>((const double*)cols[c].values + cols[c].offset, srows, m, d + c);
+            fx_sample_kernel<<<(int)std::min<int64_t>((m + 255) / 256, 256), 256, 0, s>>>((const double*)cols[c].values + cols[c].offset, srows, m, d + c, FxSampleRange{});
         VNM_HIP(hipGetLastError());
         VNM_HIP(hipMemcpyAsync(got, d, 8 * FXN_MAXV, hipMemcpyDeviceToHost, s));
         VNM_HIP(hipStreamSynchronize(s));
diff --git a/vinum_amd/csrc/vnm_agg_routes.inc b/vinum_amd/csrc/vnm_agg_routes.inc
--- a/vinum_amd/csrc/vnm_agg_routes.inc
+++ b/vinum_amd/csrc/vnm_agg_routes.inc
@@ -85,8 +85,11 @@
     if constexpr (!PV) {
         if (r.pairs == 4) return ring_scatter_pairs<FR, CT, HV, PV, VN, FX, W32, 4>(r, d);
     }
-    if (r.pairs >= 2) return ring_scatter_pairs<FR, CT, HV, PV, VN, FX, W32, 2>(r, d);
-    return ring_scatter_pairs<FR, CT, HV, PV, VN, FX, W32, 1>(r, d);
+    if constexpr (ring_reads_w32<FR, CT, FX>()) return ring_scatter_pairs<FR, CT, HV, PV, VN, FX, W32, 2>(r, d);
+    else {
+        if (r.pairs >= 2) return ring_scatter_pairs<FR, CT, HV, PV, VN, FX, W32, 2>(r, d);
+        return ring_scatter_pairs<FR, CT, HV, PV, VN, FX, W32, 1>(r, d);
+    }
 }
 
 
@@ -723,7 +726,9 @@
     int c8_cb, c8_sub;
     bool fx;
     double fx_q;
+    int fx_qe;
     bool w32, w32_1;
+    int64_t fx_bias;
     int grid1, split2;
     int64_t cap1, cap2;
     bool c16_1;
@@ -754,15 +759,26 @@
     PoolScope pool;
     unsigned long long* d = (unsigned long long*)pool.take(64);
     if (!d) return 1;
-    unsigned long long got = 0;
-    VNM_HIP(hipMemsetAsync(d, 0, 8, s));
+    unsigned long long got3[3] = {0, 0, 0};
+    VNM_HIP(hipMemsetAsync(d, 0, 24, s));
     const int64_t srows = h->segs_active ? (*h->segs_active)[0].nrows : nrows;
     const int64_t m = std::min<int64_t>(srows, 1 << 16);
-    fx_sample_kernel<<<(int)std::min<int64_t>((m + 255) / 256, 256), 256, 0, s>>>((const double*)a.cols[0].values + a.cols[0].offset, srows, m, d);
+    FxSampleRange rg{};
+    rg.out = d + 1;
+    rg.has_pred = h->pred_set ? 1 : 0; rg.op = a.p.op; rg.thr = a.p.dval;
+    if (h->pred_set && !a.hot_pred_is_v) {
+        const vnm_dcol& pc = h->segs_active ? (*h->segs_active)[0].pred : a.pred;
+        rg.pp = (const double*)pc.values + pc.offset;
+    }
+    if (!h->segs_active && a.cols[0].validity) { rg.vvalid = a.cols[0].validity; rg.voff = a.cols[0].offset; }
+    fx_sample_kernel<<<(int)std::min<int64_t>((m + 255) / 256, 256), 256, 0, s>>>((const double*)a.cols[0].values + a.cols[0].offset, srows, m, d, rg);
     VNM_HIP(hipGetLastError());
-    VNM_HIP(hipMemcpyAsync(&got, d, 8, hipMemcpyDeviceToHost, s));
+    VNM_HIP(hipMemcpyAsync(got3, d, 24, hipMemcpyDeviceToHost, s));
     VNM_HIP(hipStreamSynchronize(s));
+    const unsigned long long got = got3[0];
     const uint32_t xinv = (uint32_t)got, xexp = (uint32_t)(got >> 32);
+    h->fx_ranged = got3[1] != 0 && got3[2] != 0;
+    if (h->fx_ranged) { h->fx_smin = dec_f64(~(uint64_t)got3[1]); h->fx_smax = dec_f64((uint64_t)got3[2]); }
     if (xinv == 0 && xexp == 0) { h->fx_state = 1; h->fx_qe = -16; }
     else if (xexp < 2047) {
         const int L = (int)(0xFFFFu - xinv) - 1075, E = (int)xexp - 1022;
@@ -772,11 +788,27 @@
         if (spare >= 0) {
             int qe = L - spare / 2;
             if (qe > 0) qe = 0;
-            if (qe >= -1000 && E - qe <= room) { h->fx_state = 1; h->fx_qe = qe; h->fx_narrow = narrow; }
+            if (qe >= -1000 && E - qe <= room) { h->fx_state = 1; h->fx_qe = qe; h->fx_narrow = narrow; h->fx_low = L; }
         }
     }
     if (getenv("VNM_AGG_TRACE")) fprintf(stderr, "[agg] fixed-point entries: sample says %s (qe %d)\n", h->fx_state == 1 ? "yes" : "no", h->fx_qe);
     return 0;
+}
+
+bool plan_biased_words(const vnm_agg* h, const AggArgs& a, int rem_bits, int* qe, int64_t* bias) {
+    if (!h->fx_narrow1 || !h->fx_ranged || env_i64("VNM_DENSE_FX_NARROW1", 1) == 0) return false;
+    const int room = 32 - rem_bits;
+    if (room < 1 || room > 31) return false;
+    const double lim = 262144.0;
+    const bool bound = h->pred_set && a.hot_pred_is_v && (a.p.op == VNM_GT || a.p.op == VNM_GE) && std::isfinite(a.p.dval);
+    for (int q = h->fx_qe; q <= std::min(h->fx_low, 0); q++) {
+        const double lo = std::ldexp(h->fx_smin, -q), hi = std::ldexp(h->fx_smax, -q);
+        if (!(std::fabs(lo) < lim && std::fabs(hi) < lim)) continue;
+        const double proved = bound ? std::floor(std::ldexp(a.p.dval, -q)) : lo;
+        const double b = bound && proved <= lo && hi - proved < std::ldexp(1.0, room) && std::fabs(proved) <= lim ? proved : lo;
+        if (hi - b < std::ldexp(1.0, room)) { *qe = q; *bias = (int64_t)b; return true; }
+    }
+    return false;
 }
 
 int plan_dense_geometry(const vnm_agg* h, const AggArgs& a, int64_t nrows, const DGenArgs& g, DensePlan* p) {
@@ -841,9 +873,16 @@
     if (fx_small && levels == 1) fsplits = 1;
     p->fsplits = fsplits;
     p->fx = fx_ok && fsplits == 1 && !p->count8 && tb >= (fx_small ? 7 : 11) && tb <= 13;
-    p->fx_q = p->fx ? std::ldexp(1.0, h->fx_qe) : 0.0;
+    p->fx_qe = h->fx_qe;
     p->w32 = p->fx && h->fx_narrow;
     p->w32_1 = p->w32 && levels == 1;
+    p->fx_bias = 0;
+    if (p->w32 && levels == 2 && plan_biased_words(h, a, mp.bits - p1, &p->fx_qe, &p->fx_bias)) {
+        p->w32_1 = true;
+        cap1 = (cap1 + 31) & ~31LL; if (((cap1 / 32) & 1) == 0) cap1 += 32;
+        p->cap1 = cap1;
+    }
+    p->fx_q = p->fx ? std::ldexp(1.0, p->fx_qe) : 0.0;
     if (levels == 2) {
         const int64_t per_pg = (int64_t)grid1 * rows_per_wg / np1 / split2;
         int64_t cap2 = ((per_pg / np2 + per_pg / np2 / 4 + 256) + 15) & ~15LL;
@@ -860,7 +899,7 @@
     p->rcap1 = p->w32_1 ? ring_cap_w32(np1) : ((use_ring & 1) && !a.has_expr ? ring_cap_for(np1, p->fx ? 8 : (has_val ? 8 : 0) + (p->c16_1 ? 2 : 4)) : 0);
     if (levels == 2) p->rcap2 = p->fx ? (p->w32 ? ring_cap_w32(np2) : ring_cap_for(np2, 8)) : ((use_ring & 2) ? ring_cap_for(np2, (has_val ? 8 : 0) + 2) : 0);
     p->ring_pairs1 = (int)env_i64("VNM_DENSE_RING_PAIRS", 4);
-    if (p->fx && levels == 2 && getenv("VNM_DENSE_RING_PAIRS") == nullptr) p->ring_pairs1 = 2;
+    if (p->fx && levels == 2 && !p->w32_1 && getenv("VNM_DENSE_RING_PAIRS") == nullptr) p->ring_pairs1 = 2;
     p->ring_pairs2 = levels == 2 ? (int)env_i64("VNM_DENSE_RING_PAIRS2", p->fx && p->w32 ? 4 : 2) : 0;
     return 0;
 }
@@ -945,8 +984,10 @@
     d1.nt_store = (int)env_i64("VNM_DENSE_NT", p.levels == 2 && p.np2 >= 256 ? 1 : 0) & 1;
     d1.ready_list = (int)env_i64("VNM_DENSE_READY_LIST", 1) & 1;
     d1.flags = b.flags; d1.spill = b.spill; d1.spill_cap = p.spill_cap;
-    d1.fx_q = p.fx_q; d1.fx_inv_q = p.fx ? std::ldexp(1.0, -h->fx_qe) : 0.0;
+    d1.fx_q = p.fx_q; d1.fx_inv_q = p.fx ? std::ldexp(1.0, -p.fx_qe) : 0.0;
+    d1.fx_biased = p.w32_1 && p.levels == 2 ? 1 : 0; d1.fx_bias = p.fx_bias;
     d1.fx_lim = p.w32 ? (1LL << 18) - 1 : 2147483647LL;
+    if (d1.fx_biased) { const int64_t lim0 = d1.fx_lim >> (p.fx_qe - h->fx_qe); d1.fx_dlo = -lim0 - p.fx_bias; d1.fx_dhi = lim0 - p.fx_bias; }
     if (p.vn) { d1.vvalid = a.cols[0].validity; d1.voff = a.cols[0].offset; d1.nspill = b.nspill; d1.nspill_cap = p.nspill_cap; }
     if (h->kn_valid) {
         if (ensure_table(h, 1024, s, true)) return 1;
@@ -983,11 +1024,13 @@
     d2.nt_store = ((int)env_i64("VNM_DENSE_NT", 0) >> 1) & 1;
     d2.ready_list = ((int)env_i64("VNM_DENSE_READY_LIST", 1) >> 1) & 1;
     d2.fx_q = d1.fx_q; d2.fx_inv_q = d1.fx_inv_q; d2.fx_lim = d1.fx_lim;
+    d2.fx_biased = d1.fx_biased; d2.fx_bias = d1.fx_bias;
     const int grid2 = p.np1 * p.split2;
     const RingLaunch r{grid2, p.rcap2, ring_sub_tile_pairs(p.ring_pairs2, false, p.ring_limit, p.np2, p.rcap2, p.w32), p.ring_limit, false, false, s};
     {
         KernelTimer timer("agg_part_scatter2", s);
-        if (p.fx) VNM_TRY(pick_bool(p.w32, [&](auto w32) { return ring_scatter<false, uint32_t, true, false, false, true, decltype(w32)::value>(r, d2); }));
+        if (p.fx && p.w32 && p.w32_1) VNM_TRY((ring_scatter<false, uint32_t, true, false, false, true, true>(r, d2)));
+        else if (p.fx) VNM_TRY(pick_bool(p.w32, [&](auto w32) { return ring_scatter<false, uint64_t, true, false, false, true, decltype(w32)::value>(r, d2); }));
         else if (p.rcap2) VNM_TRY(pick_bool(p.has_val, [&](auto hv) { return ring_scatter<false, uint16_t, decltype(hv)::value, false, false>(r, d2); }));
         else VNM_TRY(pick_bool(p.has_val, [&](auto hv) { dpart_scatter_kernel<false, uint16_t, decltype(hv)::value><<<grid2, PT_BLOCK, 0, s>>>(d2); return 0; }));
     }
@@ -1065,6 +1108,14 @@
         fprintf(stderr, "[agg] dense: bits %d tb %d levels %d p1 %d p2 %d -> scatter fail %llu spilled %llu, final pass deferred (bound %lld)\n",
                 mp.bits, p.tb, p.levels, p.p1, p.p2, fl0[0], fl0[2], (long long)p.dstride);
     if (p.fx && fl0[7]) {
+        if (p.levels == 2 && p.w32_1) {
+            h->fx_narrow1 = false;
+            const bool wide = (fl0[7] & 2) != 0;
+            if (wide) { h->fx_narrow = false; h->fx_qe = std::max(h->fx_qe - 6, -1000); }
+            route_note("dense:fixed_point_misfit", "a value outside 2^%d * [%lld, %lld + 2^%d): the batch is redone with 64-bit words out of %s", p.fx_qe, (long long)p.fx_bias,
+                       (long long)p.fx_bias, 32 - (mp.bits - p.p1), wide ? "both levels" : "the first level");
+            return DENSE_REDO;
+        }
         if (h->fx_narrow) {
             h->fx_narrow = false;
             h->fx_qe = std::max(h->fx_qe - 6, -1000);
@@ -1076,7 +1127,9 @@
         return DENSE_REDO;
     }
     if (fl0[0]) return 2;
-    if (p.fx) route_note("dense:fixed_point", "%s entry words, quantum 2^%d", p.w32 ? (p.levels == 1 ? "4-byte" : "8-byte, then 4-byte") : "8-byte", h->fx_qe);
+    if (p.fx) route_note("dense:fixed_point", "%s entry words, quantum 2^%d", p.w32 ? (p.levels == 1 ? "4-byte" : (p.w32_1 ? "4-byte, then 4-byte" : "8-byte, then 4-byte")) : "8-byte", p.fx_qe);
+    if (p.fx && p.levels == 2 && p.w32_1)
+        route_note("dense:fixed_point_narrow1", "level 1 wrote 4-byte words: (m - %lld) in %d bits above %d remainder bits, quantum 2^%d", (long long)p.fx_bias, 32 - (mp.bits - p.p1), mp.bits - p.p1, p.fx_qe);
     if (fold_null_rows(h, a, b.flags, s)) return 1;
     b.pool.done(b.rk); b.pool.done(b.ra);
     if (fl0[2]) { b.pool.keep(b.spill); *spill_out = b.spill; *n_spill_out = (int64_t)fl0[2]; }
```
